# ooowedyn/InkLayer

Hardware: AMD Instinct MI355X
Metric: sketches/sec end-to-end (GroundingDINO+SAM) at 1024x1024 (higher is better)
Workload: dtype f16 (MFMA, f32 accumulate; f32 residual/norm/softmax; split-f16 = fp32-grade operands for patch-embed, neck, mask decoder)

## Files before the change

include/inklayer_hip.h:

```cpp
#ifndef INKLAYER_HIP_H
#define INKLAYER_HIP_H

#include <stdint.h>

#ifdef __cplusplus
extern "C" {
#endif

#define INK_ABI_VERSION 7
int ink_abi_version(void);

typedef struct InkGemm {
  const void* A;
  const void* W;
  const float* bias;
  const float* col_scale;
  const float* residual;
  const int32_t* row_map;
  void* C;
  int32_t M, N, K;
  int32_t lda, ldw, ldr, ldc;
  int32_t act;
  int32_t c_f16;
} InkGemm;
#define INK_ACT_NONE 0
#define INK_ACT_GELU 1
#define INK_ACT_RELU 2
int ink_gemm_f16(const InkGemm* p, void* stream);
int ink_gemm_set_variant(int32_t v);
int ink_gemm_query_variant(int32_t M, int32_t N, int32_t K);

int ink_layernorm_rows(const float* x, int64_t ldx, const float* gamma, const float* beta,
                       float eps, const int32_t* gather, int32_t rows_out, int32_t C,
                       void* out_f16, float* out_f32, int64_t ldo, int32_t act, int32_t split,
                       const float* add, int64_t ld_add, const int32_t* add_batch_rows, int32_t rows_per_batch,
                       void* stream);

int ink_add_cvt_f16(const float* a, const float* b, int64_t n_b, void* out_f16, int64_t n,
                    void* stream);
int ink_add_split_f16(const float* a, const float* b, int64_t n_b, void* out_f16, int64_t n, int32_t C,
                      void* stream);
int ink_add_f32(const float* a, const float* b, int64_t n_b, float* out, int64_t n, void* stream);

typedef struct InkAttn {
  const void* Q; const void* K; const void* V;
  void* O;
  int64_t ldq, ldk, ldv, ldo;
  int32_t n_batch, n_heads, n_q, n_k, head_dim;
  float scale;
  int32_t bias_mode;
  int32_t grid_w;
  const int32_t* q_batch_rows;
  const int32_t* kv_batch_rows;
  const float* rel_h; const float* rel_w;
  const void* rel_aug;
  const float* dense_bias; const float* dense_mask;
  int32_t n_mask; int32_t rel_f16;
  const int32_t* tok_rows;
  const void* pad_k; const void* pad_v;
} InkAttn;
int ink_flash_attn(const InkAttn* p, void* stream);

int ink_relpos_bias64_f16(const void* Q, int64_t ldq, const float* rel_pos_h, const float* rel_pos_w, int32_t n_batch,
                          int32_t n_heads, int32_t head_dim, float scale, void* out_h_f16, void* out_w_f16, void* stream);

int ink_relpos_bias(const void* Q, int64_t ldq, const float* rel_pos_h, const float* rel_pos_w,
                    int32_t S, int32_t n_batch, int32_t n_heads, int32_t head_dim, float scale,
                    const int32_t* tok_rows, float* out_h, float* out_w, void* out_aug_f16,
                    void* stream);

int ink_sam_patchify(const void* image_u8, int32_t h, int32_t w, int32_t L, int32_t P,
                     const float* mean3, const float* std3, int32_t chan_reverse, int32_t split,
                     void* out_f16, void* stream);

int ink_resize_bilinear_u8(const void* src_u8, int32_t h, int32_t w, void* dst_u8, int32_t oh, int32_t ow,
                           const int32_t* xbounds, const int32_t* xcoef, int32_t kx,
                           const int32_t* ybounds, const int32_t* ycoef, int32_t ky, void* tmp_u8,
                           void* stream);

int ink_im2col3x3_f16(const void* in_f16, int32_t B, int32_t H, int32_t W, int32_t C, void* out_f16,
                      void* stream);

int ink_sam_pe_encode(const float* coords01, const float* gauss, int32_t N, int32_t F,
                      const float* add, int32_t n_add, float* out, void* stream);

int ink_sam_prompt_tokens(const float* points, const int32_t* labels, int32_t n_pts, int32_t pad, const float* boxes,
                          const float* gauss, int32_t F, const float* point_emb, const float* not_a_point,
                          const float* out_tok, float input_size, int32_t P, float* out, void* stream);

int ink_sam_mask_embed(const float* mask, const float* emb, const int32_t* emb_rows, const float* params,
                       int32_t n_params, float eps, int32_t P, int32_t g, float* keys, void* split_f16, void* stream);

int ink_sam_mask_logits(const float* up, const float* hyper, int32_t n, int32_t g, int32_t C,
                        float* out, void* stream);

int ink_sam_postprocess(const float* low, int32_t n, int32_t S, int32_t L, int32_t in_h,
                        int32_t in_w, int32_t out_h, int32_t out_w, float thr, void* out_u8,
                        float* out_logits, void* stream);

int ink_ms_deform_attn_forward(const float* value, const int64_t* spatial_shapes_host,
                               const int64_t* level_start_index_host, const float* sampling_loc,
                               const float* attn_weight, int32_t B, int32_t S, int32_t M, int32_t C,
                               int32_t Q, int32_t L, int32_t P, int32_t im2col_step, float* out,
                               void* stream);

int ink_ms_deform_attn_forward_dev(const void* value, const int64_t* spatial_shapes,
                                   const int64_t* level_start_index, const void* sampling_loc,
                                   const void* attn_weight, int32_t dtype, int32_t B, int32_t S, int32_t M,
                                   int32_t C, int32_t Q, int32_t L, int32_t P, int32_t im2col_step,
                                   void* out, void* stream);
int ink_ms_deform_attn_backward_dev(const void* value, const int64_t* spatial_shapes,
                                    const int64_t* level_start_index, const void* sampling_loc,
                                    const void* attn_weight, const void* grad_output, int32_t dtype,
                                    int32_t B, int32_t S, int32_t M, int32_t C, int32_t Q, int32_t L,
                                    int32_t P, int32_t im2col_step, void* grad_value,
                                    void* grad_sampling_loc, void* grad_attn_weight, void* stream);

int ink_msda_fused(const void* value_f16, const float* proj, int64_t ldp, const float* ref,
                   int32_t ref_dim, int64_t ref_q_stride, int64_t ref_b_stride,
                   const int32_t* shapes_host, int32_t B, int32_t S, int32_t Q, void* out_f16,
                   void* stream);

int ink_swin_patchify(const void* image_u8, int32_t h, int32_t w, const float* mean3,
                      const float* std3, void* out_f16, void* stream);

int ink_layernorm_merge4(const float* x, int64_t ldx, const float* gamma, const float* beta, float eps,
                         const int32_t* gather4, int32_t rows, int32_t C, void* out_f16, void* stream);

int ink_groupnorm_nhwc(const float* x, int32_t B, int32_t T, int32_t C, int32_t G, const float* gamma,
                       const float* beta, float eps, float* stats_ws, float* out,
                       int64_t out_batch_stride, void* stream);

int ink_gather_rows(const float* x, int64_t ldx, int64_t x_batch_rows, const int32_t* idx,
                    int64_t idx_batch_stride, int32_t rows_per_batch, int32_t B, int32_t C,
                    void* out_f16, float* out_f32, void* stream);

int ink_biattn_fusion(const void* QV_f16, const void* KL_f16, int32_t B, int32_t S, int32_t T, int32_t E,
                      float scale, float* scores_ws, float* stats_ws, float* partial_ws, int32_t chunk,
                      void* out_v_f16, void* out_l_f16, void* stream);

int ink_attn_fewkeys(const void* Q, int64_t ldq, const void* K, int64_t ldk, const void* V, int64_t ldv,
                     int32_t B, int32_t n_q, int32_t n_k, int32_t n_heads, int32_t head_dim, float scale,
                     const uint8_t* blocked, const int32_t* q_batch_rows, const float* q_add, int32_t io_f32, void* O,
                     int64_t ldo, void* stream);

int ink_attn_fewq(const void* Q, int64_t ldq, const void* K, int64_t ldk, const void* V, int64_t ldv,
                  int32_t n_batch, int32_t n_q, int32_t n_k, int32_t n_heads, int32_t head_dim, float scale,
                  const int32_t* q_batch_rows, const int32_t* kv_batch_rows, const float* k_add, int32_t io_f32, void* O,
                  int64_t ldo, void* stream);

int ink_biattn_colstats(const float* scores, int32_t B, int32_t S, int32_t HT, float* part_ws, float* stats, void* stream);

int ink_fusion_fold_workspace(int32_t B, int32_t S, int64_t* out_floats);
int ink_fusion_fold(float* v_f32, int32_t B, int32_t S, const float* lnv_g, const float* lnv_b, float eps,
                    const float* text_k_f32, const float* text_vl_f32, int64_t ld_text, int32_t T, const void* Wq_f16,
                    const float* bq, const void* Wvv_f16, const float* bvv, const void* Wo_f16, const float* bo,
                    const float* gamma_v, float scale, float* ws, void* out_l_f16, const float* pos, void* out16_pos,
                    void* out16, void* stream);

int ink_sam_upscale_pack(const void* ws_f16, void* blob_f16, void* stream);
int ink_sam_upscale_tail(const float* u0, int64_t ld_tok, int32_t n, int32_t g, const float* ln_g, const float* ln_b, float eps,
                         const void* blob_f16, const float* b3, const float* hyper, int32_t n_masks, float* low,
                         void* stream);

int ink_proj256_ln_pack(const void* ws_f16, void* blob_f16, void* stream);
int ink_proj256_ln(const float* a_f32, const void* blob_f16, const float* bias, const float* res_f32,
                   const int32_t* res_batch_rows, int32_t rows_per_batch, const float* ln_g, const float* ln_b, float eps,
                   int64_t rows, float* out_f32, void* out_split_f16, void* stream);

int ink_ffn256_pack_bytes(int32_t hid, int32_t with_pre, int64_t* out_bytes);
int ink_ffn256_pack(const void* w1_f16, const float* b1, const void* w2_f16, int32_t hid, const void* wpre_f16, void* blob,
                    void* stream);
int ink_ffn256_fused(const void* x_f16, int64_t ldx, const float* res_f32, const void* blob, const float* b2,
                     const float* ln_g, const float* ln_b, float eps, int32_t M, int32_t hid, const float* pre_bias,
                     const float* pre_ln_g, const float* pre_ln_b, float* out_f32, void* stream);

int ink_topk_rowmax(const float* logits, int32_t B, int32_t S, int32_t T, int32_t K, int32_t* out_idx,
                    float* out_val, void* cand_ws, void* stream);

int ink_sine_embed4(const float* ref, const float* dim_t, int32_t N, void* out_f16, void* stream);

int ink_box_refine(const float* delta, int64_t ldd, const float* ref, int32_t N, int32_t ref_is_logit,
                   float* out, void* stream);

int ink_mask_cleanup_workspace_ints(int32_t n, int32_t H, int32_t W, int32_t k, int64_t* out_ints);
int ink_mask_cleanup(const void* masks_u8, int32_t n, int32_t H, int32_t W, int32_t k, int32_t area_threshold,
                     double aspect_threshold, void* tmp_a_u8, void* tmp_b_u8, int32_t* workspace, void* out_u8,
                     void* stream);

int ink_mask_sketch_iou_counts(const void* masks_u8, const void* sketch_rgb_u8, int32_t n, int32_t H, int32_t W,
                               void* bits_ws_u64, int32_t* counts, void* stream);

int ink_sam_amg_stats(const float* low, int32_t n, const int32_t* index, int32_t m, const int32_t* m_dev, int32_t S,
                      int32_t L, int32_t in_h, int32_t in_w, int32_t crop_h, int32_t crop_w, double thr, double offset,
                      int32_t x0, int32_t y0, int32_t orig_h, int32_t orig_w, int32_t* table, void* planes_u64,
                      float* out_logits, void* stream);

int ink_mask_rle_counts(const void* planes_u64, const int32_t* select, int32_t k, int32_t H, int32_t W,
                        int32_t* n_counts, void* stream);
int ink_mask_rle_write(const void* planes_u64, const int32_t* select, int32_t k, int32_t H, int32_t W,
                       const int32_t* offsets, int32_t* counts, void* stream);

int ink_mask_small_regions_workspace_ints(int32_t k, int32_t H, int32_t W, int64_t* out_ints);
int ink_mask_small_regions(const void* planes_u64, int32_t k, int32_t H, int32_t W, int32_t min_area, int32_t holes,
                           void* tmp_planes_u64, int32_t* workspace, void* out_planes_u64, int32_t* changed, void* stream);

int ink_box_nms(const float* boxes, const float* scores, int32_t n, float iou_threshold, void* workspace_u64,
                int32_t* keep, int32_t* n_keep, void* stream);

int ink_refine_sketch_planes(const void* rgb_u8, int32_t H, int32_t W, void* planes4_u64, int32_t* max_ws, void* stream);

int ink_bitplane_pack(const void* img_u8, int32_t n, int32_t H, int32_t W, int32_t thresh, void* planes_u64, void* stream);

int ink_refine_depth_samples(const void* mask_planes, int32_t n, const float* depth, const int32_t* pts_yx, int32_t P,
                             int32_t H, int32_t W, float* vals, void* inside_u8, void* stream);

int ink_refine_pair_tables(const void* mask_planes, const void* sketch_planes4, int32_t n, int32_t H, int32_t W,
                           const int32_t* rect, void* dil_ws_planes, int32_t* pair, int32_t* per_mask,
                           int32_t* sketch_area, void* stream);

int ink_refine_composite(const void* mask_planes, const int32_t* order, int32_t n_ranks, int32_t H, int32_t W,
                         void* label_u8, int32_t* hist256, void* stream);

int ink_refine_relabel_clean(const void* label_u8, const void* map256_u8, int32_t H, int32_t W, void* out_label_u8,
                             void* stream);

int ink_refine_grow_workspace(int32_t H, int32_t W, int64_t* plane_words, int64_t* cc_ints);
int ink_refine_grow(const void* label_u8, const void* sketch_planes4, int32_t H, int32_t W, void* planes_ws,
                    int32_t* cc_ws, int32_t* flags256, void* out_label_u8, int32_t* bbox256x4, int32_t* unl_yx,
                    int32_t unl_cap, int32_t* unl_count, void* stream);

int ink_refine_query_dists(const void* label_u8, const int32_t* q_yx, const void* cand256_bits, int32_t Q, int32_t H,
                           int32_t W, int32_t* d2_Qx256, void* stream);

int ink_refine_finalize(void* label_u8, const int32_t* assign_yxl, int32_t A, const void* sketch_planes4, int32_t H,
                        int32_t W, void* planes_ws3, void* extra_plane, int32_t* extra_count, void* stream);

int ink_host_sparse_sample(const uint8_t* rgb_u8, int32_t H, int32_t W, int32_t* out_yx, int32_t cap, int32_t* count);
int ink_host_assign_unlabeled(const int32_t* q_yx, int32_t Q, const int32_t* boxes, int32_t nb, const int32_t* box2mask,
                              const int32_t* d2, const uint8_t* nonempty, int32_t n_masks, int32_t* out_label);

int ink_depth_patchify(const void* image_u8, int32_t H, int32_t W, int32_t nh, int32_t nw, int32_t P, int32_t KP,
                       const double* mean3, const double* std3, int32_t chan_reverse, void* out_f16, void* stream);

int ink_resize_bilinear_ac_nhwc(const float* in, int32_t B, int32_t h, int32_t w, int32_t C, int32_t H, int32_t W,
                                float* out_f32, void* out_f16, void* stream);

int ink_im2col3x3_ex_f16(const void* in_f16, int32_t B, int32_t H, int32_t W, int32_t C, int32_t stride, int32_t relu,
                         void* out_f16, void* stream);

#ifdef __cplusplus
}
#endif
#endif
```

inklayer_amd/_lib.py:

```python
from __future__ import annotations

import ctypes as C
import os
from pathlib import Path

_LIB_PATH = Path(__file__).resolve().parent / "lib" / "libinklayer_hip.so"
_lib = None

c_void_p, c_int, c_i64, c_float = C.c_void_p, C.c_int32, C.c_int64, C.c_float


class InkGemm(C.Structure):
    _fields_ = [
        ("A", c_void_p), ("W", c_void_p), ("bias", c_void_p), ("col_scale", c_void_p),
        ("residual", c_void_p), ("row_map", c_void_p), ("C", c_void_p),
        ("M", c_int), ("N", c_int), ("K", c_int),
        ("lda", c_int), ("ldw", c_int), ("ldr", c_int), ("ldc", c_int),
        ("act", c_int), ("c_f16", c_int),
    ]


class InkAttn(C.Structure):
    _fields_ = [
        ("Q", c_void_p), ("K", c_void_p), ("V", c_void_p), ("O", c_void_p),
        ("ldq", c_i64), ("ldk", c_i64), ("ldv", c_i64), ("ldo", c_i64),
        ("n_batch", c_int), ("n_heads", c_int), ("n_q", c_int), ("n_k", c_int),
        ("head_dim", c_int), ("scale", c_float), ("bias_mode", c_int), ("grid_w", c_int),
        ("q_batch_rows", c_void_p), ("kv_batch_rows", c_void_p),
        ("rel_h", c_void_p), ("rel_w", c_void_p), ("rel_aug", c_void_p),
        ("dense_bias", c_void_p), ("dense_mask", c_void_p), ("n_mask", c_int), ("rel_f16", c_int),
        ("tok_rows", c_void_p), ("pad_k", c_void_p), ("pad_v", c_void_p),
    ]


SIGNATURES = {
    "ink_abi_version": [],
    "ink_gemm_f16": [C.POINTER(InkGemm), c_void_p],
    "ink_gemm_set_variant": [c_int],
    "ink_gemm_query_variant": [c_int, c_int, c_int],
    "ink_layernorm_rows": [c_void_p, c_i64, c_void_p, c_void_p, c_float, c_void_p, c_int, c_int,
                           c_void_p, c_void_p, c_i64, c_int, c_int, c_void_p, c_i64, c_void_p, c_int, c_void_p],
    "ink_add_split_f16": [c_void_p, c_void_p, c_i64, c_void_p, c_i64, c_int, c_void_p],
    "ink_add_cvt_f16": [c_void_p, c_void_p, c_i64, c_void_p, c_i64, c_void_p],
    "ink_add_f32": [c_void_p, c_void_p, c_i64, c_void_p, c_i64, c_void_p],
    "ink_flash_attn": [C.POINTER(InkAttn), c_void_p],
    "ink_sam_patchify": [c_void_p, c_int, c_int, c_int, c_int, C.POINTER(c_float), C.POINTER(c_float),
                         c_int, c_int, c_void_p, c_void_p],
    "ink_im2col3x3_f16": [c_void_p, c_int, c_int, c_int, c_int, c_void_p, c_void_p],
    "ink_resize_bilinear_u8": [c_void_p, c_int, c_int, c_void_p, c_int, c_int, c_void_p, c_void_p, c_int,
                               c_void_p, c_void_p, c_int, c_void_p, c_void_p],
    "ink_sam_pe_encode": [c_void_p, c_void_p, c_int, c_int, c_void_p, c_int, c_void_p, c_void_p],
    "ink_sam_mask_logits": [c_void_p, c_void_p, c_int, c_int, c_int, c_void_p, c_void_p],
    "ink_sam_prompt_tokens": [c_void_p, c_void_p, c_int, c_int, c_void_p, c_void_p, c_int, c_void_p, c_void_p,
                              c_void_p, c_float, c_int, c_void_p, c_void_p],
    "ink_sam_mask_embed": [c_void_p, c_void_p, c_void_p, c_void_p, c_int, c_float, c_int, c_int, c_void_p, c_void_p,
                           c_void_p],
    "ink_sam_postprocess": [c_void_p, c_int, c_int, c_int, c_int, c_int, c_int, c_int, c_float,
                            c_void_p, c_void_p, c_void_p],
    "ink_sam_amg_stats": [c_void_p, c_int, c_void_p, c_int, c_void_p, c_int, c_int, c_int, c_int, c_int, c_int, C.c_double,
                          C.c_double, c_int, c_int, c_int, c_int, c_void_p, c_void_p, c_void_p, c_void_p],
    "ink_mask_rle_counts": [c_void_p, c_void_p, c_int, c_int, c_int, c_void_p, c_void_p],
    "ink_mask_rle_write": [c_void_p, c_void_p, c_int, c_int, c_int, c_void_p, c_void_p, c_void_p],
    "ink_mask_small_regions_workspace_ints": [c_int, c_int, c_int, C.POINTER(c_i64)],
    "ink_mask_small_regions": [c_void_p, c_int, c_int, c_int, c_int, c_int, c_void_p, c_void_p, c_void_p, c_void_p,
                               c_void_p],
    "ink_box_nms": [c_void_p, c_void_p, c_int, c_float, c_void_p, c_void_p, c_void_p, c_void_p],
    "ink_ms_deform_attn_forward": [c_void_p, C.POINTER(c_i64), C.POINTER(c_i64), c_void_p, c_void_p, c_int,
                                   c_int, c_int, c_int, c_int, c_int, c_int, c_int, c_void_p, c_void_p],
    "ink_ms_deform_attn_forward_dev": [c_void_p, c_void_p, c_void_p, c_void_p, c_void_p, c_int, c_int, c_int, c_int,
                                       c_int, c_int, c_int, c_int, c_int, c_void_p, c_void_p],
    "ink_ms_deform_attn_backward_dev": [c_void_p, c_void_p, c_void_p, c_void_p, c_void_p, c_void_p, c_int, c_int, c_int,
                                        c_int, c_int, c_int, c_int, c_int, c_int, c_void_p, c_void_p, c_void_p,
                                        c_void_p],
    "ink_msda_fused": [c_void_p, c_void_p, c_i64, c_void_p, c_int, c_i64, c_i64, C.POINTER(c_int), c_int,
                       c_int, c_int, c_void_p, c_void_p],
    "ink_swin_patchify": [c_void_p, c_int, c_int, C.POINTER(c_float), C.POINTER(c_float), c_void_p, c_void_p],
    "ink_layernorm_merge4": [c_void_p, c_i64, c_void_p, c_void_p, c_float, c_void_p, c_int, c_int, c_void_p,
                             c_void_p],
    "ink_groupnorm_nhwc": [c_void_p, c_int, c_int, c_int, c_int, c_void_p, c_void_p, c_float, c_void_p,
                           c_void_p, c_i64, c_void_p],
    "ink_gather_rows": [c_void_p, c_i64, c_i64, c_void_p, c_i64, c_int, c_int, c_int, c_void_p, c_void_p,
                        c_void_p],
    "ink_biattn_fusion": [c_void_p, c_void_p, c_int, c_int, c_int, c_int, c_float, c_void_p, c_void_p,
                          c_void_p, c_int, c_void_p, c_void_p, c_void_p],
    "ink_biattn_colstats": [c_void_p, c_int, c_int, c_int, c_void_p, c_void_p, c_void_p],
    "ink_fusion_fold_workspace": [c_int, c_int, C.POINTER(c_i64)],
    "ink_relpos_bias64_f16": [c_void_p, c_i64, c_void_p, c_void_p, c_int, c_int, c_int, c_float, c_void_p, c_void_p, c_void_p],
    "ink_proj256_ln_pack": [c_void_p, c_void_p, c_void_p],
    "ink_proj256_ln": [c_void_p, c_void_p, c_void_p, c_void_p, c_void_p, c_int, c_void_p, c_void_p, c_float, c_i64, c_void_p,
                       c_void_p, c_void_p],
    "ink_sam_upscale_pack": [c_void_p, c_void_p, c_void_p],
    "ink_sam_upscale_tail": [c_void_p, c_i64, c_int, c_int, c_void_p, c_void_p, c_float, c_void_p, c_void_p, c_void_p,
                             c_int, c_void_p, c_void_p],
    "ink_ffn256_pack_bytes": [c_int, c_int, C.POINTER(c_i64)],
    "ink_ffn256_pack": [c_void_p, c_void_p, c_void_p, c_int, c_void_p, c_void_p, c_void_p],
    "ink_ffn256_fused": [c_void_p, c_i64, c_void_p, c_void_p, c_void_p, c_void_p, c_void_p, c_float, c_int, c_int,
                         c_void_p, c_void_p, c_void_p, c_void_p, c_void_p],
    "ink_fusion_fold": [c_void_p, c_int, c_int, c_void_p, c_void_p, c_float, c_void_p, c_void_p, c_i64, c_int, c_void_p,
                        c_void_p, c_void_p, c_void_p, c_void_p, c_void_p, c_void_p, c_float, c_void_p, c_void_p, c_void_p,
                        c_void_p, c_void_p, c_void_p],
    "ink_attn_fewkeys": [c_void_p, c_i64, c_void_p, c_i64, c_void_p, c_i64, c_int, c_int, c_int, c_int, c_int,
                         c_float, c_void_p, c_void_p, c_void_p, c_int, c_void_p, c_i64, c_void_p],
    "ink_attn_fewq": [c_void_p, c_i64, c_void_p, c_i64, c_void_p, c_i64, c_int, c_int, c_int, c_int, c_int,
                      c_float, c_void_p, c_void_p, c_void_p, c_int, c_void_p, c_i64, c_void_p],
    "ink_topk_rowmax": [c_void_p, c_int, c_int, c_int, c_int, c_void_p, c_void_p, c_void_p, c_void_p],
    "ink_sine_embed4": [c_void_p, c_void_p, c_int, c_void_p, c_void_p],
    "ink_box_refine": [c_void_p, c_i64, c_void_p, c_int, c_int, c_void_p, c_void_p],
    "ink_mask_cleanup_workspace_ints": [c_int, c_int, c_int, c_int, C.POINTER(c_i64)],
    "ink_mask_cleanup": [c_void_p, c_int, c_int, c_int, c_int, c_int, C.c_double, c_void_p, c_void_p, c_void_p,
                         c_void_p, c_void_p],
    "ink_mask_sketch_iou_counts": [c_void_p, c_void_p, c_int, c_int, c_int, c_void_p, c_void_p, c_void_p],
    "ink_refine_sketch_planes": [c_void_p, c_int, c_int, c_void_p, c_void_p, c_void_p],
    "ink_bitplane_pack": [c_void_p, c_int, c_int, c_int, c_int, c_void_p, c_void_p],
    "ink_refine_depth_samples": [c_void_p, c_int, c_void_p, c_void_p, c_int, c_int, c_int, c_void_p, c_void_p, c_void_p],
    "ink_refine_pair_tables": [c_void_p, c_void_p, c_int, c_int, c_int, c_void_p, c_void_p, c_void_p, c_void_p,
                               c_void_p, c_void_p],
    "ink_refine_composite": [c_void_p, c_void_p, c_int, c_int, c_int, c_void_p, c_void_p, c_void_p],
    "ink_refine_relabel_clean": [c_void_p, c_void_p, c_int, c_int, c_void_p, c_void_p],
    "ink_refine_grow_workspace": [c_int, c_int, C.POINTER(c_i64), C.POINTER(c_i64)],
    "ink_refine_grow": [c_void_p, c_void_p, c_int, c_int, c_void_p, c_void_p, c_void_p, c_void_p, c_void_p, c_void_p,
                        c_int, c_void_p, c_void_p],
    "ink_refine_query_dists": [c_void_p, c_void_p, c_void_p, c_int, c_int, c_int, c_void_p, c_void_p],
    "ink_refine_finalize": [c_void_p, c_void_p, c_int, c_void_p, c_int, c_int, c_void_p, c_void_p, c_void_p, c_void_p],
    "ink_host_sparse_sample": [c_void_p, c_int, c_int, c_void_p, c_int, c_void_p],
    "ink_host_assign_unlabeled": [c_void_p, c_int, c_void_p, c_int, c_void_p, c_void_p, c_void_p, c_int, c_void_p],
    "ink_depth_patchify": [c_void_p, c_int, c_int, c_int, c_int, c_int, c_int, C.POINTER(C.c_double), C.POINTER(C.c_double),
                           c_int, c_void_p, c_void_p],
    "ink_resize_bilinear_ac_nhwc": [c_void_p, c_int, c_int, c_int, c_int, c_int, c_int, c_void_p, c_void_p, c_void_p],
    "ink_im2col3x3_ex_f16": [c_void_p, c_int, c_int, c_int, c_int, c_int, c_int, c_void_p, c_void_p],
    "ink_relpos_bias": [c_void_p, c_i64, c_void_p, c_void_p, c_int, c_int, c_int, c_int, c_float,
                        c_void_p, c_void_p, c_void_p, c_void_p, c_void_p],
}


class InkLayerHipError(RuntimeError):
    pass


def lib_path() -> Path:
    return Path(os.environ.get("INKLAYER_HIP_LIB", _LIB_PATH))


def lib() -> C.CDLL:
    global _lib
    if _lib is None:
        p = lib_path()
        if not p.exists():
            raise InkLayerHipError(
                f"{p} not found: build it with `python -m inklayer_amd.build` "
                "(there is no CPU/eager fallback for the InkLayer hot path)")
        try:
            import torch
        except ImportError:
            pass
        l = C.CDLL(str(p))
        for name, argtypes in SIGNATURES.items():
            fn = getattr(l, name)
            fn.argtypes = argtypes
            fn.restype = C.c_int
        _lib = l
    return _lib


def check(rc: int, what: str) -> None:
    if rc != 0:
        raise InkLayerHipError(f"{what} failed: " + {1: "bad argument", 2: "HIP launch error"}.get(rc, str(rc)))
```

inklayer_amd/build.py:

```python
from __future__ import annotations

import os
import subprocess
import sys
from concurrent.futures import ThreadPoolExecutor
from pathlib import Path

ROOT = Path(__file__).resolve().parent
CSRC = ROOT / "csrc"
LIBDIR = ROOT / "lib"
OBJDIR = LIBDIR / "obj"
LIB = LIBDIR / "libinklayer_hip.so"
HIPCC = os.environ.get("HIPCC", "/opt/rocm/bin/hipcc")
FLAGS = ["--offload-arch=gfx950", "-O3", "-std=c++17", "-fPIC", "-ffp-contract=off",
         "-mllvm", "-amdgpu-mfma-vgpr-form",

         "-Wall", "-Wno-unused-function", "-Wno-unused-variable"]


def _newest_header() -> float:
    hs = list(CSRC.glob("*.h")) + list((ROOT.parent / "include").glob("*.h"))
    return max(h.stat().st_mtime for h in hs)


NO_SPILL = {"ffn_fused.hip", "proj_ln.hip", "amg.hip"}


def _check_no_spill(src: Path, remarks: str) -> None:
    name = None
    for line in remarks.splitlines():
        if "Function Name:" in line:
            name = line.split("Function Name:")[1].split("[")[0].strip()
        elif "ScratchSize [bytes/lane]:" in line:
            n = int(line.split("ScratchSize [bytes/lane]:")[1].split("[")[0])
            if n != 0:
                raise RuntimeError(f"{src.name}: kernel {name} spills ({n} bytes of scratch per lane) - the kernels of "
                                   f"this file must stay in registers (see NO_SPILL); reduce register pressure")


def _compile(src: Path, force: bool, hdr_time: float) -> Path:
    obj = OBJDIR / (src.stem + ".o")
    if (not force and obj.exists() and obj.stat().st_mtime > src.stat().st_mtime
            and obj.stat().st_mtime > hdr_time):
        return obj
    guard = src.name in NO_SPILL
    cmd = [HIPCC, *FLAGS, *(["-Rpass-analysis=kernel-resource-usage", "-fno-caret-diagnostics"] if guard else []), "-c", str(src), "-o", str(obj)]
    r = subprocess.run(cmd, capture_output=True, text=True)
    if r.returncode != 0:
        raise RuntimeError(f"hipcc failed for {src.name}:\n{r.stdout}\n{r.stderr}")
    err = r.stderr
    if guard:
        try:
            _check_no_spill(src, err)
        except RuntimeError:
            obj.unlink(missing_ok=True)
            raise
        err = "\n".join(l for l in err.splitlines()
                        if "kernel-resource-usage" not in l and not l.startswith("In file included from"))
    if err.strip():
        sys.stderr.write(err)
    return obj


def build(force: bool = False, verbose: bool = True) -> Path:
    OBJDIR.mkdir(parents=True, exist_ok=True)
    srcs = sorted(CSRC.glob("*.hip"))
    if not srcs:
        raise RuntimeError("no HIP sources found")
    hdr_time = _newest_header()
    with ThreadPoolExecutor(max_workers=min(8, len(srcs))) as ex:
        objs = list(ex.map(lambda s: _compile(s, force, hdr_time), srcs))
    if (force or not LIB.exists()
            or any(o.stat().st_mtime > LIB.stat().st_mtime for o in objs)):
        cmd = [HIPCC, "--offload-arch=gfx950", "-shared", "-fPIC", "-o", str(LIB),
               *map(str, objs)]
        r = subprocess.run(cmd, capture_output=True, text=True)
        if r.returncode != 0:
            raise RuntimeError(f"link failed:\n{r.stdout}\n{r.stderr}")
    if verbose:
        print(f"[inklayer_amd.build] {LIB} ({LIB.stat().st_size >> 10} KiB, {len(srcs)} sources)")
    return LIB


if __name__ == "__main__":
    build(force="--force" in sys.argv)
```

inklayer_amd/ops.py:

```python
from __future__ import annotations

import ctypes as C
from typing import Optional, Sequence, Tuple

import torch

from . import _lib
from ._lib import InkAttn, InkGemm, check

ACT = {None: 0, "none": 0, "gelu": 1, "relu": 2}
F16, F32 = torch.float16, torch.float32


_GEMM_TRACE = None


def set_gemm_trace(lst) -> None:
    global _GEMM_TRACE
    _GEMM_TRACE = lst


_ATTN_TRACE = None


def set_attn_trace(lst) -> None:
    global _ATTN_TRACE
    _ATTN_TRACE = lst


def tracing_off() -> bool:
    return _GEMM_TRACE is None and _ATTN_TRACE is None


_raw_stream = getattr(torch._C, "_cuda_getCurrentRawStream", None)
_cur_device = getattr(torch._C, "_cuda_getDevice", None)


def _stream() -> int:
    if _raw_stream is not None and _cur_device is not None:
        return _raw_stream(_cur_device())
    return torch.cuda.current_stream().cuda_stream


def own_f32(t: torch.Tensor, dev) -> torch.Tensor:
    t = t.detach().to(dev, F32).contiguous()
    if t.untyped_storage().nbytes() > t.numel() * t.element_size():
        t = t.clone()
    return t


def _p(t: Optional[torch.Tensor]) -> Optional[int]:
    if t is None:
        return None
    assert t.is_cuda, "InkLayer HIP ops need GPU tensors (no CPU fallback)"
    return t.data_ptr()


def gemm(a: torch.Tensor, w: torch.Tensor, bias: Optional[torch.Tensor] = None, *,
         act: Optional[str] = None, residual: Optional[torch.Tensor] = None,
         col_scale: Optional[torch.Tensor] = None, row_map: Optional[torch.Tensor] = None,
         out: Optional[torch.Tensor] = None, out_dtype: torch.dtype = F32,
         out_rows: Optional[int] = None) -> torch.Tensor:
    assert a.dtype == F16 and w.dtype == F16
    assert a.dim() == 2 and w.dim() == 2 and a.stride(1) == 1 and w.stride(1) == 1
    M, K = a.shape
    N = w.shape[0]
    assert w.shape[1] == K
    p = InkGemm()
    if out is None:
        rows = out_rows if out_rows is not None else M
        out = torch.empty((rows, N), device=a.device, dtype=out_dtype)
    assert out.dim() == 2 and out.stride(1) == 1 and out.shape[1] == N
    p.A, p.W, p.C = a.data_ptr(), w.data_ptr(), out.data_ptr()
    p.bias, p.col_scale = _p(bias), _p(col_scale)
    p.residual, p.row_map = _p(residual), _p(row_map)
    if bias is not None:
        assert bias.dtype == F32 and bias.numel() == N
    if col_scale is not None:
        assert col_scale.dtype == F32 and col_scale.numel() == N
    if residual is not None:
        assert residual.dtype == F32 and residual.stride(1) == 1 and residual.shape[1] == N
        p.ldr = residual.stride(0)
    if row_map is not None:
        assert row_map.dtype == torch.int32 and row_map.numel() == M
    p.M, p.N, p.K = M, N, K
    p.lda, p.ldw, p.ldc = a.stride(0), w.stride(0), out.stride(0)
    p.act = ACT[act]
    p.c_f16 = 1 if out.dtype == F16 else 0
    assert out.dtype in (F16, F32)
    if _GEMM_TRACE is None:
        check(_lib.lib().ink_gemm_f16(C.byref(p), _stream()), "ink_gemm_f16")
    else:
        e0, e1 = torch.cuda.Event(enable_timing=True), torch.cuda.Event(enable_timing=True)
        e0.record()
        check(_lib.lib().ink_gemm_f16(C.byref(p), _stream()), "ink_gemm_f16")
        e1.record()
        _GEMM_TRACE.append((2.0 * M * N * K, e0, e1, (M, N, K, act or '-', 'res' if residual is not None else '-',
                                                      'map' if row_map is not None else '-', 'f16' if p.c_f16 else 'f32')))
    return out


def layernorm_rows(x: torch.Tensor, gamma: Optional[torch.Tensor], beta: Optional[torch.Tensor],
                   eps: float, *, gather: Optional[torch.Tensor] = None,
                   out_dtype: torch.dtype = F16, out: Optional[torch.Tensor] = None,
                   out2: Optional[torch.Tensor] = None, act: Optional[str] = None,
                   split: bool = False, add: Optional[torch.Tensor] = None,
                   add_batch_rows: Optional[torch.Tensor] = None, rows_per_batch: int = 0,
                   split_f32: Optional[torch.Tensor] = None) -> torch.Tensor:
    assert x.dtype == F32 and x.dim() == 2 and x.stride(1) == 1
    Cdim = x.shape[1]
    rows = gather.numel() if gather is not None else x.shape[0]
    wcols = 3 * Cdim if split else Cdim
    if split:
        assert out_dtype == F16 and out2 is None
    if out is None:
        out = torch.empty((rows, wcols), device=x.device, dtype=out_dtype)
    assert out.shape == (rows, wcols) and out.stride(1) == 1
    oh = out.data_ptr() if out.dtype == F16 else None
    of = out.data_ptr() if out.dtype == F32 else None
    if out2 is not None:
        assert out2.shape == out.shape and out2.stride(0) == out.stride(0) and out2.dtype != out.dtype
        if out2.dtype == F16:
            oh = out2.data_ptr()
        else:
            of = out2.data_ptr()
    if split_f32 is not None:
        assert split and out.stride(0) == 3 * Cdim and split_f32.dtype == F32 and split_f32.is_contiguous()
        assert tuple(split_f32.shape) == (rows, Cdim)
        of = split_f32.data_ptr()
    if gather is not None:
        assert gather.dtype == torch.int32
    if add is not None:
        assert gather is None and add.dtype == F32 and add.dim() == 2 and add.stride(1) == 1 and add.shape[1] == Cdim
        if add_batch_rows is not None:
            assert add_batch_rows.dtype == torch.int32 and add_batch_rows.is_cuda and rows_per_batch > 0
            assert add_batch_rows.numel() * rows_per_batch == rows
        else:
            rows_per_batch = rows
    check(_lib.lib().ink_layernorm_rows(x.data_ptr(), x.stride(0), _p(gamma), _p(beta), eps,
                                        _p(gather), rows, Cdim, oh, of, out.stride(0), ACT[act], int(split),
                                        _p(add), add.stride(0) if add is not None else 0, _p(add_batch_rows),
                                        rows_per_batch, _stream()), "ink_layernorm_rows")
    return out


def add_cvt_f16(a: torch.Tensor, b: Optional[torch.Tensor] = None,
                out: Optional[torch.Tensor] = None) -> torch.Tensor:
    assert a.dtype == F32 and a.is_contiguous()
    nb = 0
    if b is not None:
        assert b.dtype == F32 and b.is_contiguous() and a.numel() % b.numel() == 0
        nb = b.numel()
    if out is None:
        out = torch.empty(a.shape, device=a.device, dtype=F16)
    assert out.dtype == F16 and out.is_contiguous() and out.numel() == a.numel()
    check(_lib.lib().ink_add_cvt_f16(a.data_ptr(), _p(b), nb, out.data_ptr(), a.numel(), _stream()),
          "ink_add_cvt_f16")
    return out


def add_split_f16(a: torch.Tensor, b: Optional[torch.Tensor] = None) -> torch.Tensor:
    assert a.dtype == F32 and a.is_contiguous() and a.dim() == 2
    nb = 0
    if b is not None:
        assert b.dtype == F32 and b.is_contiguous() and a.numel() % b.numel() == 0
        nb = b.numel()
    R, Cn = a.shape
    out = torch.empty((R, 3 * Cn), device=a.device, dtype=F16)
    check(_lib.lib().ink_add_split_f16(a.data_ptr(), _p(b), nb, out.data_ptr(), a.numel(), Cn, _stream()),
          "ink_add_split_f16")
    return out


def split_weight(w32: torch.Tensor) -> torch.Tensor:
    w32 = w32.to(torch.float32)
    hi = w32.to(F16)
    lo = ((w32 - hi.to(torch.float32)) * 64.0).to(F16)
    return torch.cat([hi, (hi.to(torch.float32) / 64.0).to(F16), lo], dim=-1).contiguous()


def add_f32(a: torch.Tensor, b: torch.Tensor, out: Optional[torch.Tensor] = None) -> torch.Tensor:
    assert a.dtype == F32 and b.dtype == F32 and a.is_contiguous() and b.is_contiguous()
    assert a.numel() % b.numel() == 0
    if out is None:
        out = torch.empty(a.shape, device=a.device, dtype=F32)
    assert out.is_contiguous() and out.numel() == a.numel()
    check(_lib.lib().ink_add_f32(a.data_ptr(), b.data_ptr(), b.numel(), out.data_ptr(), a.numel(),
                                 _stream()), "ink_add_f32")
    return out


def flash_attn(q: torch.Tensor, k: torch.Tensor, v: torch.Tensor, *, n_batch: int, n_heads: int,
               head_dim: int, scale: float, n_q: Optional[int] = None, n_k: Optional[int] = None,
               rel_h: Optional[torch.Tensor] = None, rel_w: Optional[torch.Tensor] = None,
               rel_aug: Optional[torch.Tensor] = None, grid_w: int = 0,
               dense_bias: Optional[torch.Tensor] = None, dense_mask: Optional[torch.Tensor] = None,
               q_batch_rows: Optional[torch.Tensor] = None,
               kv_batch_rows: Optional[torch.Tensor] = None,
               tok_rows: Optional[torch.Tensor] = None, pad_k: Optional[torch.Tensor] = None,
               pad_v: Optional[torch.Tensor] = None,
               out: Optional[torch.Tensor] = None) -> torch.Tensor:
    for t in (q, k, v):
        assert t.dtype == F16 and t.dim() == 2 and t.stride(1) == 1 and t.is_cuda
    if n_q is None:
        n_q = q.shape[0] // n_batch
    if n_k is None:
        n_k = k.shape[0] // n_batch
    if tok_rows is not None:
        assert rel_aug is not None and out is not None and n_q == n_k
        assert tok_rows.dtype == torch.int32 and tok_rows.is_cuda and tok_rows.numel() == n_batch * n_q
        for t in (pad_k, pad_v):
            assert t is not None and t.dtype == F16 and t.is_contiguous() and t.numel() == n_heads * head_dim
        assert out.dtype == F16 and out.stride(1) == 1
        assert out.shape[0] * out.stride(0) * 2 < 2 ** 31 and q.shape[0] * q.stride(0) * 2 < 2 ** 32
    else:
        if out is None:
            out = torch.empty((n_batch * n_q, n_heads * head_dim), device=q.device, dtype=F16)
        assert out.dtype == F16 and out.shape[0] == n_batch * n_q and out.stride(1) == 1
    p = InkAttn()
    p.Q, p.K, p.V, p.O = q.data_ptr(), k.data_ptr(), v.data_ptr(), out.data_ptr()
    p.ldq, p.ldk, p.ldv, p.ldo = q.stride(0), k.stride(0), v.stride(0), out.stride(0)
    p.n_batch, p.n_heads, p.n_q, p.n_k, p.head_dim = n_batch, n_heads, n_q, n_k, head_dim
    p.scale = scale
    p.grid_w = grid_w
    for name, t in (("q_batch_rows", q_batch_rows), ("kv_batch_rows", kv_batch_rows)):
        if t is not None:
            assert t.dtype == torch.int32 and t.numel() == n_batch and t.is_cuda
            setattr(p, name, t.data_ptr())
    if dense_bias is not None:
        assert dense_bias.dtype == F32 and dense_bias.is_contiguous() and dense_bias.shape == (n_heads, n_q, 64)
        p.bias_mode, p.dense_bias = 3, dense_bias.data_ptr()
        if dense_mask is not None:
            assert dense_mask.dtype == F32 and dense_mask.is_contiguous() and dense_mask.shape[1:] == (n_q, 64)
            p.dense_mask, p.n_mask = dense_mask.data_ptr(), dense_mask.shape[0]
    elif rel_aug is not None:
        assert rel_aug.dtype == F16 and rel_aug.is_contiguous()
        p.bias_mode, p.rel_aug = 2, rel_aug.data_ptr()
        if tok_rows is not None:
            p.tok_rows, p.pad_k, p.pad_v = tok_rows.data_ptr(), pad_k.data_ptr(), pad_v.data_ptr()
    elif rel_h is not None:
        assert rel_h.dtype == rel_w.dtype and rel_h.dtype in (F32, F16)
        assert rel_h.is_contiguous() and rel_w.is_contiguous()
        p.bias_mode, p.rel_h, p.rel_w = 1, rel_h.data_ptr(), rel_w.data_ptr()
        p.rel_f16 = int(rel_h.dtype == F16)
    else:
        p.bias_mode = 0
    if _ATTN_TRACE is None:
        check(_lib.lib().ink_flash_attn(C.byref(p), _stream()), "ink_flash_attn")
    else:
        e0, e1 = torch.cuda.Event(enable_timing=True), torch.cuda.Event(enable_timing=True)
        e0.record()
        check(_lib.lib().ink_flash_attn(C.byref(p), _stream()), "ink_flash_attn")
        e1.record()
        _ATTN_TRACE.append((n_batch, n_heads, n_q, n_k, head_dim, int(p.bias_mode), int(out.shape[0]), e0, e1))
    return out


def relpos_bias(q: torch.Tensor, rel_pos_h: torch.Tensor, rel_pos_w: torch.Tensor, *, S: int,
                n_batch: int, n_heads: int, head_dim: int, scale: float, out=None,
                tok_rows: Optional[torch.Tensor] = None, f16_tables: bool = False):
    assert q.dtype == F16 and q.stride(1) == 1
    assert rel_pos_h.dtype == F32 and rel_pos_h.is_contiguous()
    assert rel_pos_w.dtype == F32 and rel_pos_w.is_contiguous()
    assert rel_pos_h.shape == (2 * S - 1, head_dim)
    n = n_batch * n_heads * S * S
    fn = _lib.lib().ink_relpos_bias
    if S == 64 and f16_tables:
        oh, ow = out if out is not None else (torch.empty((n, 64), device=q.device, dtype=F16),
                                              torch.empty((n, 64), device=q.device, dtype=F16))
        assert oh.dtype == F16 and ow.dtype == F16 and oh.numel() >= n * 64 and ow.numel() >= n * 64
        check(_lib.lib().ink_relpos_bias64_f16(q.data_ptr(), q.stride(0), rel_pos_h.data_ptr(), rel_pos_w.data_ptr(), n_batch,
                                               n_heads, head_dim, scale, oh.data_ptr(), ow.data_ptr(), _stream()),
              "ink_relpos_bias64_f16")
        return oh, ow
    if S == 64:
        oh, ow = out if out is not None else (torch.empty((n, 64), device=q.device, dtype=F32),
                                              torch.empty((n, 64), device=q.device, dtype=F32))
        assert oh.numel() >= n * 64 and ow.numel() >= n * 64
        check(fn(q.data_ptr(), q.stride(0), rel_pos_h.data_ptr(), rel_pos_w.data_ptr(), S, n_batch,
                 n_heads, head_dim, scale, None, oh.data_ptr(), ow.data_ptr(), None, _stream()),
              "ink_relpos_bias")
        return oh, ow
    aug = out if out is not None else torch.empty((n, 32), device=q.device, dtype=F16)
    assert aug.numel() >= n * 32
    if tok_rows is not None:
        assert tok_rows.dtype == torch.int32 and tok_rows.is_cuda and tok_rows.numel() == n_batch * S * S
    check(fn(q.data_ptr(), q.stride(0), rel_pos_h.data_ptr(), rel_pos_w.data_ptr(), S, n_batch,
             n_heads, head_dim, scale, tok_rows.data_ptr() if tok_rows is not None else None,
             None, None, aug.data_ptr(), _stream()), "ink_relpos_bias")
    return aug


def resize_bilinear_u8(image_u8: torch.Tensor, oh: int, ow: int, out: Optional[torch.Tensor] = None) -> torch.Tensor:
    from .resize import plan_for
    assert image_u8.dtype == torch.uint8 and image_u8.is_cuda and image_u8.is_contiguous()
    h, w, c = image_u8.shape
    assert c == 3
    if (oh, ow) == (h, w):
        return image_u8
    pl = plan_for(h, w, oh, ow, image_u8.device)
    if out is None:
        out = torch.empty((oh, ow, 3), device=image_u8.device, dtype=torch.uint8)
    assert out.dtype == torch.uint8 and out.is_contiguous() and tuple(out.shape) == (oh, ow, 3)
    ptr = lambda t: t.data_ptr() if t is not None else None
    check(_lib.lib().ink_resize_bilinear_u8(image_u8.data_ptr(), h, w, out.data_ptr(), oh, ow, ptr(pl.xb), ptr(pl.xk),
                                            pl.kx, ptr(pl.yb), ptr(pl.yk), pl.ky, ptr(pl.tmp), _stream()),
          "ink_resize_bilinear_u8")
    return out


def sam_patchify(image_u8: torch.Tensor, L: int, P: int, mean: Sequence[float],
                 std: Sequence[float], chan_reverse: bool, out: torch.Tensor, split: bool = False) -> torch.Tensor:
    assert image_u8.dtype == torch.uint8 and image_u8.is_cuda and image_u8.is_contiguous()
    h, w, c = image_u8.shape
    assert c == 3 and out.dtype == F16 and out.is_contiguous()
    assert out.numel() == (L // P) ** 2 * 3 * P * P * (3 if split else 1)
    m = (C.c_float * 3)(*mean)
    s = (C.c_float * 3)(*std)
    check(_lib.lib().ink_sam_patchify(image_u8.data_ptr(), h, w, L, P, m, s, int(chan_reverse), int(split),
                                      out.data_ptr(), _stream()), "ink_sam_patchify")
    return out


def im2col3x3(x: torch.Tensor, B: int, H: int, W: int, out: Optional[torch.Tensor] = None) -> torch.Tensor:
    assert x.dtype == F16 and x.is_contiguous() and x.shape[0] == B * H * W
    Cn = x.shape[1]
    if out is None:
        out = torch.empty((B * H * W, 9 * Cn), device=x.device, dtype=F16)
    check(_lib.lib().ink_im2col3x3_f16(x.data_ptr(), B, H, W, Cn, out.data_ptr(), _stream()),
          "ink_im2col3x3_f16")
    return out


def sam_pe_encode(coords01: torch.Tensor, gauss: torch.Tensor,
                  add: Optional[torch.Tensor] = None, out: Optional[torch.Tensor] = None) -> torch.Tensor:
    assert coords01.dtype == F32 and coords01.is_contiguous() and coords01.shape[-1] == 2
    assert gauss.dtype == F32 and gauss.is_contiguous() and gauss.shape[0] == 2
    N, Fd = coords01.numel() // 2, gauss.shape[1]
    if out is None:
        out = torch.empty((N, 2 * Fd), device=coords01.device, dtype=F32)
    assert out.dtype == F32 and out.is_contiguous() and tuple(out.shape) == (N, 2 * Fd)
    n_add = 0
    if add is not None:
        assert add.dtype == F32 and add.is_contiguous() and add.shape[-1] == 2 * Fd
        n_add = add.numel() // (2 * Fd)
    check(_lib.lib().ink_sam_pe_encode(coords01.data_ptr(), gauss.data_ptr(), N, Fd, _p(add), n_add,
                                       out.data_ptr(), _stream()), "ink_sam_pe_encode")
    return out


def sam_prompt_tokens(gauss: torch.Tensor, point_emb: torch.Tensor, not_a_point: torch.Tensor, out_tok: torch.Tensor,
                      input_size: float, P: int, points: Optional[torch.Tensor] = None,
                      labels: Optional[torch.Tensor] = None, boxes: Optional[torch.Tensor] = None, pad: bool = False,
                      out: Optional[torch.Tensor] = None) -> torch.Tensor:
    Fd = gauss.shape[1]
    assert gauss.dtype == F32 and gauss.is_contiguous() and gauss.shape[0] == 2
    for t, n in ((point_emb, 4), (not_a_point, 1), (out_tok, 5)):
        assert t.dtype == F32 and t.is_contiguous() and t.numel() == n * 2 * Fd
    n_pts = 0
    if points is not None:
        assert labels is not None and points.dtype == F32 and labels.dtype == torch.int32
        assert points.is_contiguous() and labels.is_contiguous() and points.dim() == 3 and points.shape[0] == P
        n_pts = points.shape[1]
        assert tuple(points.shape) == (P, n_pts, 2) and tuple(labels.shape) == (P, n_pts)
    if boxes is not None:
        assert boxes.dtype == F32 and boxes.is_contiguous() and tuple(boxes.shape) == (P, 4)
    NT = 5 + n_pts + int(pad) + (2 if boxes is not None else 0)
    if out is None:
        out = torch.empty((P, NT, 2 * Fd), device=gauss.device, dtype=F32)
    assert out.dtype == F32 and out.is_contiguous() and tuple(out.shape) == (P, NT, 2 * Fd)
    check(_lib.lib().ink_sam_prompt_tokens(_p(points), _p(labels), n_pts, int(pad), _p(boxes), _p(gauss), Fd,
                                           _p(point_emb), _p(not_a_point), _p(out_tok),
                                           float(input_size), P, _p(out), _stream()), "ink_sam_prompt_tokens")
    return out


SAM_MASK_EMBED_PARAMS = 4684


def sam_mask_embed(mask: torch.Tensor, emb: torch.Tensor, emb_rows: torch.Tensor, params: torch.Tensor, eps: float,
                   split: bool = False):
    assert mask.dtype == F32 and mask.is_contiguous() and mask.dim() == 4 and mask.shape[1] == 1
    P, S = mask.shape[0], mask.shape[2]
    assert mask.shape[3] == S and S % 4 == 0
    g = S // 4
    assert emb.dtype == F32 and emb.is_contiguous() and emb.dim() == 2 and emb.shape[1] == 256
    assert emb_rows.dtype == torch.int32 and emb_rows.is_cuda and emb_rows.numel() == P
    assert params.dtype == F32 and params.is_contiguous() and params.numel() == SAM_MASK_EMBED_PARAMS
    keys = torch.empty((P * g * g, 256), device=mask.device, dtype=F32)
    ks = torch.empty((P * g * g, 768), device=mask.device, dtype=F16) if split else None
    check(_lib.lib().ink_sam_mask_embed(_p(mask), _p(emb), _p(emb_rows), _p(params),
                                        params.numel(), eps, P, g, _p(keys), _p(ks), _stream()),
          "ink_sam_mask_embed")
    return (keys, ks) if split else keys


def sam_mask_logits(up: torch.Tensor, hyper: torch.Tensor, n: int, g: int) -> torch.Tensor:
    assert up.dtype == F32 and up.is_contiguous() and hyper.dtype == F32 and hyper.is_contiguous()
    Cn = hyper.shape[1]
    assert up.numel() == n * g * g * 16 * Cn
    out = torch.empty((n, 4 * g, 4 * g), device=up.device, dtype=F32)
    check(_lib.lib().ink_sam_mask_logits(up.data_ptr(), hyper.data_ptr(), n, g, Cn, out.data_ptr(),
                                         _stream()), "ink_sam_mask_logits")
    return out


def sam_postprocess(low: torch.Tensor, L: int, input_hw: Tuple[int, int], orig_hw: Tuple[int, int],
                    thr: float = 0.0, want_logits: bool = False):
    assert low.dtype == F32 and low.is_contiguous() and low.dim() == 3
    n, S, _ = low.shape
    oh, ow = orig_hw
    out = torch.empty((n, oh, ow), device=low.device, dtype=torch.uint8)
    lg = torch.empty((n, oh, ow), device=low.device, dtype=F32) if want_logits else None
    check(_lib.lib().ink_sam_postprocess(low.data_ptr(), n, S, L, input_hw[0], input_hw[1], oh, ow,
                                         thr, out.data_ptr(), _p(lg), _stream()),
          "ink_sam_postprocess")
    return (out, lg) if want_logits else out


NMS_MAX_BOXES = 4096


def sam_amg_stats(low: torch.Tensor, L: int, input_hw: Tuple[int, int], crop_hw: Tuple[int, int], thr: float,
                  offset: float, xy0: Tuple[int, int] = (0, 0), orig_hw: Optional[Tuple[int, int]] = None,
                  index: Optional[torch.Tensor] = None, count: Optional[torch.Tensor] = None,
                  want_logits: bool = False):
    assert low.dtype == F32 and low.is_contiguous() and low.dim() == 3
    n, S, _ = low.shape
    ch, cw = crop_hw
    oh, ow = orig_hw if orig_hw is not None else crop_hw
    if index is not None:
        assert index.dtype == torch.int32 and index.is_cuda and index.is_contiguous() and index.dim() == 1
    if count is not None:
        assert count.dtype == torch.int32 and count.is_cuda and count.numel() == 1
    m = n if index is None else index.numel()
    hp = -(-oh // 64)
    table = torch.empty((m, 8), device=low.device, dtype=torch.int32)
    planes = torch.empty((m, ow, hp), device=low.device, dtype=torch.int64)
    lg = torch.empty((m, ch, cw), device=low.device, dtype=F32) if want_logits else None
    if m > 0:
        check(_lib.lib().ink_sam_amg_stats(low.data_ptr(), n, _p(index), m, _p(count), S, L, input_hw[0], input_hw[1],
                                           ch, cw, thr, offset, xy0[0], xy0[1], oh, ow, table.data_ptr(),
                                           planes.data_ptr(), _p(lg), _stream()), "ink_sam_amg_stats")
    return (table, planes, lg) if want_logits else (table, planes)


def mask_rle(planes: torch.Tensor, H: int, W: int, select: Optional[torch.Tensor] = None):
    assert planes.dtype == torch.int64 and planes.is_cuda and planes.is_contiguous()
    assert planes.dim() == 3 and tuple(planes.shape[1:]) == (W, -(-H // 64))
    if select is not None:
        assert select.dtype == torch.int32 and select.is_cuda and select.is_contiguous() and select.dim() == 1
    k = planes.shape[0] if select is None else select.numel()
    if k == 0:
        return []
    nc = torch.empty((k,), device=planes.device, dtype=torch.int32)
    check(_lib.lib().ink_mask_rle_counts(planes.data_ptr(), _p(select), k, H, W, nc.data_ptr(), _stream()),
          "ink_mask_rle_counts")
    sizes = nc.cpu()
    ends = torch.cumsum(sizes.long(), 0)
    total = int(ends[-1])
    assert total < 2 ** 31
    offs = (ends - sizes).to(torch.int32).to(planes.device)
    counts = torch.empty((total,), device=planes.device, dtype=torch.int32)
    check(_lib.lib().ink_mask_rle_write(planes.data_ptr(), _p(select), k, H, W, offs.data_ptr(), counts.data_ptr(),
                                        _stream()), "ink_mask_rle_write")
    return [c.tolist() for c in torch.split(counts.cpu(), sizes.tolist())]


def box_nms(boxes: torch.Tensor, scores: torch.Tensor, iou_threshold: float) -> torch.Tensor:
    assert boxes.dtype == F32 and boxes.is_cuda and boxes.is_contiguous() and boxes.dim() == 2 and boxes.shape[1] == 4
    assert scores.dtype == F32 and scores.is_cuda and scores.is_contiguous() and scores.shape == boxes.shape[:1]
    n = boxes.shape[0]
    if n > NMS_MAX_BOXES:
        raise ValueError(f"box_nms serves at most {NMS_MAX_BOXES} boxes, got {n}")
    if n == 0:
        return torch.empty((0,), device=boxes.device, dtype=torch.int64)
    ws = torch.empty((n * (-(-n // 64) + 3),), device=boxes.device, dtype=torch.int64)
    keep = torch.empty((n + 1,), device=boxes.device, dtype=torch.int32)
    check(_lib.lib().ink_box_nms(boxes.data_ptr(), scores.data_ptr(), n, iou_threshold, ws.data_ptr(), keep.data_ptr(),
                                 keep[n:].data_ptr(), _stream()), "ink_box_nms")
    host = keep.cpu()
    return host[:int(host[n])].long().to(boxes.device)


def pack_col_planes(masks: torch.Tensor) -> torch.Tensor:
    assert masks.is_cuda and masks.dim() == 3 and masks.dtype in (torch.bool, torch.uint8)
    k, H, W = masks.shape
    t = masks.to(torch.uint8).transpose(1, 2).contiguous()
    planes = torch.empty((k, W, -(-H // 64)), device=masks.device, dtype=torch.int64)
    if k:
        check(_lib.lib().ink_bitplane_pack(t.data_ptr(), k, W, H, 0, planes.data_ptr(), _stream()), "ink_bitplane_pack")
    return planes


def remove_small_regions(planes: torch.Tensor, H: int, W: int, min_area: int, max_workspace_bytes: int = 1 << 29,
                         modes: Sequence[str] = ("holes", "islands")) -> Tuple[torch.Tensor, torch.Tensor]:
    assert planes.dtype == torch.int64 and planes.is_cuda and planes.is_contiguous()
    assert planes.dim() == 3 and tuple(planes.shape[1:]) == (W, -(-H // 64))
    k = planes.shape[0]
    out = torch.empty_like(planes)
    changed = torch.zeros((k,), device=planes.device, dtype=torch.int32)
    if k == 0:
        return out, changed.bool()
    L = _lib.lib()
    one = C.c_int64(0)
    check(L.ink_mask_small_regions_workspace_ints(1, H, W, C.byref(one)), "ink_mask_small_regions_workspace_ints")
    chunk = max(1, min(k, max_workspace_bytes // (4 * one.value)))
    need = C.c_int64(0)
    check(L.ink_mask_small_regions_workspace_ints(chunk, H, W, C.byref(need)), "ink_mask_small_regions_workspace_ints")
    ws = torch.empty((need.value,), device=planes.device, dtype=torch.int32)
    tmp = torch.empty_like(planes[:chunk])
    flag = torch.empty((chunk,), device=planes.device, dtype=torch.int32)
    for a in range(0, k, chunk):
        n = min(chunk, k - a)
        src, dst = planes[a:a + n], out[a:a + n]
        for j, mode in enumerate(modes):
            assert mode in ("holes", "islands")
            holes = int(mode == "holes")
            check(L.ink_mask_small_regions((dst if j else src).data_ptr(), n, H, W, int(min_area), holes,
                                           tmp.data_ptr(), ws.data_ptr(), dst.data_ptr(), flag.data_ptr(), _stream()),
                  "ink_mask_small_regions")
            changed[a:a + n] |= flag[:n]
    return out, changed.bool()


_MSDA_DTYPE = {F32: 0, torch.float64: 1}


def _msda_check(value: torch.Tensor, spatial_shapes, level_start_index, sampling_loc: torch.Tensor,
                attn_weight: torch.Tensor, im2col_step: int, *grads: torch.Tensor):
    ss = spatial_shapes if isinstance(spatial_shapes, torch.Tensor) else torch.as_tensor(spatial_shapes)
    ls = level_start_index if isinstance(level_start_index, torch.Tensor) else torch.as_tensor(level_start_index)
    floats = (value, sampling_loc, attn_weight, *grads)
    if value.dtype not in _MSDA_DTYPE:
        raise ValueError(f"ms_deform_attn: value must be float32 or float64, got {value.dtype}")
    if any(t.dtype != value.dtype for t in floats):
        raise ValueError("ms_deform_attn: value, sampling_loc, attn_weight (and grad_output) must share one dtype, got "
                         + ", ".join(str(t.dtype) for t in floats))
    if ss.dtype != torch.int64 or ls.dtype != torch.int64:
        raise ValueError(f"ms_deform_attn: spatial_shapes / level_start_index must be int64, got {ss.dtype} / {ls.dtype}")
    if not all(t.is_cuda for t in floats):
        raise ValueError("ms_deform_attn: value, sampling_loc, attn_weight must be GPU tensors (no CPU path)")
    if not all(t.is_contiguous() for t in (*floats, ss, ls)):
        raise ValueError("ms_deform_attn: every tensor must be contiguous")
    if value.dim() != 4 or sampling_loc.dim() != 6 or sampling_loc.shape[-1] != 2:
        raise ValueError("ms_deform_attn: value must be [B,S,M,C] and sampling_loc [B,Q,M,L,P,2]")
    B, S, M, Cn = value.shape
    _, Q, _, L, P, _ = sampling_loc.shape
    if (tuple(sampling_loc.shape[:3]) != (B, Q, M) or tuple(attn_weight.shape) != (B, Q, M, L, P)
            or tuple(ss.shape) != (L, 2) or tuple(ls.shape) != (L,)):
        raise ValueError("ms_deform_attn: inconsistent shapes of value / spatial_shapes / level_start_index / "
                         "sampling_loc / attn_weight")
    if any(tuple(g.shape) != (B, Q, M * Cn) for g in grads):
        raise ValueError(f"ms_deform_attn: grad_output must be [B,Q,M*C] = {(B, Q, M * Cn)}")
    step = min(B, im2col_step)
    if im2col_step <= 0 or B % step != 0:
        raise ValueError(f"ms_deform_attn: im2col_step ({im2col_step}) must divide batch ({B})")
    for t, name in ((ss, "spatial_shapes"), (ls, "level_start_index")):
        if t.is_cuda and t.device != value.device:
            raise ValueError(f"ms_deform_attn: {name} is on {t.device}, value on {value.device}")
    return ss, ls, (B, S, M, Cn, Q, L, P)


def _msda_device_tables(ss: torch.Tensor, ls: torch.Tensor, S: int, dev) -> Tuple[torch.Tensor, torch.Tensor]:
    if ss.is_cuda and ls.is_cuda:
        return ss, ls
    if ss.is_cuda or ls.is_cuda:
        raise ValueError("ms_deform_attn: spatial_shapes and level_start_index must both be host or both be device tensors")
    hw = [int(h) * int(w) for h, w in ss.tolist()]
    starts = [sum(hw[:i]) for i in range(len(hw))]
    if min(int(v) for v in ss.reshape(-1).tolist()) <= 0 or sum(hw) != S or ls.tolist() != starts:
        raise ValueError(f"ms_deform_attn: spatial_shapes {ss.tolist()} / level_start_index {ls.tolist()} do not "
                         f"describe the {S} rows of value")
    return ss.to(dev), ls.to(dev)


def ms_deform_attn_forward(value: torch.Tensor, spatial_shapes, level_start_index,
                           sampling_loc: torch.Tensor, attn_weight: torch.Tensor,
                           im2col_step: int = 64) -> torch.Tensor:
    ss, ls, (B, S, M, Cn, Q, L, P) = _msda_check(value, spatial_shapes, level_start_index, sampling_loc, attn_weight,
                                                 im2col_step)
    out = torch.empty((B, Q, M * Cn), device=value.device, dtype=value.dtype)
    if not ss.is_cuda and not ls.is_cuda and value.dtype == F32 and Cn == 32 and L <= 8:
        sl = [int(v) for v in ss.reshape(-1).tolist()]
        ll = [int(v) for v in ls.tolist()]
        check(_lib.lib().ink_ms_deform_attn_forward(
            value.data_ptr(), (C.c_int64 * len(sl))(*sl), (C.c_int64 * len(ll))(*ll), sampling_loc.data_ptr(),
            attn_weight.data_ptr(), B, S, M, Cn, Q, L, P, im2col_step, out.data_ptr(), _stream()),
            "ink_ms_deform_attn_forward")
        return out
    ss, ls = _msda_device_tables(ss, ls, S, value.device)
    check(_lib.lib().ink_ms_deform_attn_forward_dev(
        value.data_ptr(), ss.data_ptr(), ls.data_ptr(), sampling_loc.data_ptr(), attn_weight.data_ptr(),
        _MSDA_DTYPE[value.dtype], B, S, M, Cn, Q, L, P, im2col_step, out.data_ptr(), _stream()),
        "ink_ms_deform_attn_forward_dev")
    return out


def ms_deform_attn_backward(value: torch.Tensor, spatial_shapes, level_start_index, sampling_loc: torch.Tensor,
                            attn_weight: torch.Tensor, grad_output: torch.Tensor, im2col_step: int = 64):
    ss, ls, (B, S, M, Cn, Q, L, P) = _msda_check(value, spatial_shapes, level_start_index, sampling_loc, attn_weight,
                                                 im2col_step, grad_output)
    ss, ls = _msda_device_tables(ss, ls, S, value.device)
    grad_value = torch.empty_like(value)
    grad_loc = torch.empty_like(sampling_loc)
    grad_aw = torch.empty_like(attn_weight)
    check(_lib.lib().ink_ms_deform_attn_backward_dev(
        value.data_ptr(), ss.data_ptr(), ls.data_ptr(), sampling_loc.data_ptr(), attn_weight.data_ptr(),
        grad_output.data_ptr(), _MSDA_DTYPE[value.dtype], B, S, M, Cn, Q, L, P, im2col_step, grad_value.data_ptr(),
        grad_loc.data_ptr(), grad_aw.data_ptr(), _stream()), "ink_ms_deform_attn_backward_dev")
    return grad_value, grad_loc, grad_aw


class _MSDeformAttnFunction(torch.autograd.Function):

    @staticmethod
    def forward(ctx, value, spatial_shapes, level_start_index, sampling_loc, attn_weight, im2col_step):
        ctx.im2col_step = im2col_step
        ctx.save_for_backward(value, spatial_shapes, level_start_index, sampling_loc, attn_weight)
        return ms_deform_attn_forward(value, spatial_shapes, level_start_index, sampling_loc, attn_weight, im2col_step)

    @staticmethod
    @torch.autograd.function.once_differentiable
    def backward(ctx, grad_output):
        value, spatial_shapes, level_start_index, sampling_loc, attn_weight = ctx.saved_tensors
        gv, gl, ga = ms_deform_attn_backward(value, spatial_shapes, level_start_index, sampling_loc, attn_weight,
                                             grad_output.contiguous(), ctx.im2col_step)
        return gv, None, None, gl, ga, None


def ms_deform_attn(value: torch.Tensor, spatial_shapes, level_start_index, sampling_loc: torch.Tensor,
                   attn_weight: torch.Tensor, im2col_step: int = 64) -> torch.Tensor:
    ss = spatial_shapes if isinstance(spatial_shapes, torch.Tensor) else torch.as_tensor(spatial_shapes)
    ls = level_start_index if isinstance(level_start_index, torch.Tensor) else torch.as_tensor(level_start_index)
    return _MSDeformAttnFunction.apply(value, ss, ls, sampling_loc, attn_weight, im2col_step)


def msda_fused(value16: torch.Tensor, proj: torch.Tensor, ref: torch.Tensor, shapes: Sequence[Tuple[int, int]],
               B: int, Q: int, ref_batched: bool, out: Optional[torch.Tensor] = None) -> torch.Tensor:
    assert value16.dtype == F16 and value16.is_contiguous() and proj.dtype == F32 and proj.stride(1) == 1
    assert ref.dtype == F32 and ref.is_contiguous()
    S = value16.shape[0] // B
    d = ref.shape[-1]
    if out is None:
        out = torch.empty((B * Q, 256), device=value16.device, dtype=F16)
    flat = [v for hw in shapes for v in hw]
    check(_lib.lib().ink_msda_fused(value16.data_ptr(), proj.data_ptr(), proj.stride(0), ref.data_ptr(), d, d,
                                    Q * d if ref_batched else 0, (C.c_int32 * 8)(*flat), B, S, Q,
                                    out.data_ptr(), _stream()), "ink_msda_fused")
    return out


def swin_patchify(image_u8: torch.Tensor, mean: Sequence[float], std: Sequence[float], out: torch.Tensor):
    assert image_u8.dtype == torch.uint8 and image_u8.is_cuda and image_u8.is_contiguous()
    h, w, c = image_u8.shape
    assert c == 3 and out.dtype == F16 and out.is_contiguous() and out.numel() == -(-h // 4) * -(-w // 4) * 64
    check(_lib.lib().ink_swin_patchify(image_u8.data_ptr(), h, w, (C.c_float * 3)(*mean), (C.c_float * 3)(*std),
                                       out.data_ptr(), _stream()), "ink_swin_patchify")
    return out


def layernorm_merge4(x: torch.Tensor, gamma, beta, eps: float, gather4: torch.Tensor,
                     out: Optional[torch.Tensor] = None) -> torch.Tensor:
    assert x.dtype == F32 and x.stride(1) == 1 and gather4.dtype == torch.int32 and gather4.is_contiguous()
    rows, Cn = gather4.shape[0], x.shape[1]
    if out is None:
        out = torch.empty((rows, 4 * Cn), device=x.device, dtype=F16)
    assert out.dtype == F16 and out.is_contiguous() and tuple(out.shape) == (rows, 4 * Cn)
    check(_lib.lib().ink_layernorm_merge4(x.data_ptr(), x.stride(0), gamma.data_ptr(), beta.data_ptr(), eps,
                                          gather4.data_ptr(), rows, Cn, out.data_ptr(), _stream()),
          "ink_layernorm_merge4")
    return out


def groupnorm_nhwc(x: torch.Tensor, B: int, T: int, G: int, gamma, beta, eps: float, out: torch.Tensor,
                   out_batch_stride: int) -> None:
    assert x.dtype == F32 and x.is_contiguous() and out.dtype == F32
    Cn = x.shape[1]
    ws = torch.empty(B * G * 2, device=x.device, dtype=F32)
    check(_lib.lib().ink_groupnorm_nhwc(x.data_ptr(), B, T, Cn, G, gamma.data_ptr(), beta.data_ptr(), eps,
                                        ws.data_ptr(), out.data_ptr(), out_batch_stride, _stream()),
          "ink_groupnorm_nhwc")


def gather_rows(x: torch.Tensor, idx: torch.Tensor, B: int, rows_per_batch: int, *, x_batch_rows: int,
                idx_batch_stride: int, out_dtype=F16, out: Optional[torch.Tensor] = None) -> torch.Tensor:
    assert x.dtype == F32 and x.stride(1) == 1 and idx.dtype == torch.int32 and idx.is_cuda
    Cn = x.shape[1]
    if out is None:
        out = torch.empty((B * rows_per_batch, Cn), device=x.device, dtype=out_dtype)
    out_dtype = out.dtype
    assert out_dtype in (F16, F32) and out.is_contiguous() and tuple(out.shape) == (B * rows_per_batch, Cn)
    oh = out.data_ptr() if out_dtype == F16 else None
    of = out.data_ptr() if out_dtype == F32 else None
    check(_lib.lib().ink_gather_rows(x.data_ptr(), x.stride(0), x_batch_rows, idx.data_ptr(), idx_batch_stride,
                                     rows_per_batch, B, Cn, oh, of, _stream()), "ink_gather_rows")
    return out


def biattn_fusion(qv16: torch.Tensor, kl16: torch.Tensor, B: int, S: int, T: int, scale: float,
                  chunk: int = 128):
    assert qv16.dtype == F16 and qv16.is_contiguous() and kl16.dtype == F16 and kl16.is_contiguous()
    E = qv16.shape[1] // 2
    dev = qv16.device
    nchunk = -(-S // chunk)
    scores = torch.empty(B * S * 4 * T, device=dev, dtype=F32)
    stats = torch.empty(B * 4 * T * 2, device=dev, dtype=F32)
    partial = torch.empty(B * 4 * nchunk * T * 256, device=dev, dtype=F32)
    out_v = torch.empty((B * S, E), device=dev, dtype=F16)
    out_l = torch.empty((B * T, E), device=dev, dtype=F16)
    check(_lib.lib().ink_biattn_fusion(qv16.data_ptr(), kl16.data_ptr(), B, S, T, E, scale, scores.data_ptr(),
                                       stats.data_ptr(), partial.data_ptr(), chunk, out_v.data_ptr(),
                                       out_l.data_ptr(), _stream()), "ink_biattn_fusion")
    return out_v, out_l


def fusion_fold(v: torch.Tensor, B: int, S: int, lnv_g: torch.Tensor, lnv_b: torch.Tensor, eps: float,
                text_kv: torch.Tensor, T: int, Wqv: torch.Tensor, bqv: torch.Tensor, Wo: torch.Tensor, bo: torch.Tensor,
                gamma_v: torch.Tensor, scale: float, pos: Optional[torch.Tensor] = None,
                out16_pos: Optional[torch.Tensor] = None, out16: Optional[torch.Tensor] = None) -> torch.Tensor:
    for t in (out16, out16_pos):
        assert t is None or (t.dtype == F16 and t.is_contiguous() and tuple(t.shape) == (B * S, 256))
    assert out16_pos is None or (pos is not None and pos.dtype == F32 and pos.is_contiguous() and tuple(pos.shape) == (S, 256))
    assert v.dtype == F32 and v.is_contiguous() and tuple(v.shape) == (B * S, 256)
    assert text_kv.dtype == F32 and text_kv.stride(1) == 1 and tuple(text_kv.shape) == (B * T, 2048)
    assert Wqv.dtype == F16 and Wqv.is_contiguous() and tuple(Wqv.shape) == (2048, 256) and bqv.dtype == F32
    assert Wo.dtype == F16 and Wo.is_contiguous() and tuple(Wo.shape) == (256, 1024)
    need = C.c_int64(0)
    check(_lib.lib().ink_fusion_fold_workspace(B, S, C.byref(need)), "ink_fusion_fold_workspace")
    ws = torch.empty(need.value, device=v.device, dtype=F32)
    out_l = torch.empty((B * T, 1024), device=v.device, dtype=F16)
    check(_lib.lib().ink_fusion_fold(v.data_ptr(), B, S, lnv_g.data_ptr(), lnv_b.data_ptr(), eps, text_kv.data_ptr(),
                                     text_kv[:, 1024:].data_ptr(), text_kv.stride(0), T, Wqv.data_ptr(), bqv.data_ptr(),
                                     Wqv[1024:].data_ptr(), bqv[1024:].data_ptr(), Wo.data_ptr(), bo.data_ptr(),
                                     gamma_v.data_ptr(), scale, ws.data_ptr(), out_l.data_ptr(), _p(pos), _p(out16_pos),
                                     _p(out16), _stream()),
          "ink_fusion_fold")
    return out_l


def proj256_ln_pack(ws: torch.Tensor) -> torch.Tensor:
    assert ws.dtype == F16 and ws.is_contiguous() and tuple(ws.shape) == (256, 384)
    blob = torch.empty(3 * 64 * 64 * 8, device=ws.device, dtype=F16)
    check(_lib.lib().ink_proj256_ln_pack(ws.data_ptr(), blob.data_ptr(), _stream()), "ink_proj256_ln_pack")
    return blob


def proj256_ln(a: torch.Tensor, blob: torch.Tensor, bias: torch.Tensor, res: torch.Tensor, ln_g: torch.Tensor,
               ln_b: torch.Tensor, eps: float, *, res_batch_rows: Optional[torch.Tensor] = None, rows_per_batch: int = 0,
               want_f32: bool = True, want_split: bool = True):
    R = int(a.shape[0])
    assert a.dtype == F32 and a.is_contiguous() and tuple(a.shape) == (R, 128)
    assert blob.dtype == F16 and blob.numel() == 3 * 64 * 64 * 8
    assert res.dtype == F32 and res.is_contiguous() and res.shape[1] == 256
    assert all(t.dtype == F32 and t.is_contiguous() and t.numel() == 256 for t in (bias, ln_g, ln_b))
    if res_batch_rows is not None:
        assert res_batch_rows.dtype == torch.int32 and res_batch_rows.is_cuda and rows_per_batch > 0
        assert res_batch_rows.numel() * rows_per_batch == R
    else:
        assert res.shape[0] == R
    of = torch.empty((R, 256), device=a.device, dtype=F32) if want_f32 else None
    osp = torch.empty((R, 768), device=a.device, dtype=F16) if want_split else None
    check(_lib.lib().ink_proj256_ln(a.data_ptr(), blob.data_ptr(), bias.data_ptr(), res.data_ptr(), _p(res_batch_rows),
                                    rows_per_batch, ln_g.data_ptr(), ln_b.data_ptr(), eps, R, _p(of), _p(osp), _stream()),
          "ink_proj256_ln")
    return of, osp


def sam_upscale_pack(ws: torch.Tensor) -> torch.Tensor:
    assert ws.dtype == F16 and ws.is_contiguous() and tuple(ws.shape) == (128, 192)
    blob = torch.empty(4 * 12 * 64 * 8, device=ws.device, dtype=F16)
    check(_lib.lib().ink_sam_upscale_pack(ws.data_ptr(), blob.data_ptr(), _stream()), "ink_sam_upscale_pack")
    return blob


def sam_upscale_tail(u0: torch.Tensor, n: int, g: int, ln_g: torch.Tensor, ln_b: torch.Tensor, eps: float,
                     blob: torch.Tensor, b3: torch.Tensor, hyper: torch.Tensor) -> torch.Tensor:
    if u0.shape[1] == 64:
        assert u0.is_contiguous() and u0.shape[0] == n * g * g * 4
        u0 = u0.view(n * g * g, 256)
    assert u0.dtype == F32 and u0.stride(1) == 1 and tuple(u0.shape) == (n * g * g, 256) and u0.stride(0) % 4 == 0
    assert blob.dtype == F16 and blob.numel() == 4 * 12 * 64 * 8 and b3.dtype == F32 and b3.numel() == 128
    assert hyper.dtype == F32 and hyper.is_contiguous() and hyper.dim() == 3 and hyper.shape[0] == n and hyper.shape[2] == 32
    assert ln_g.dtype == F32 and ln_b.dtype == F32 and ln_g.numel() == 64 and ln_b.numel() == 64
    M = hyper.shape[1]
    low = torch.empty((n, M, 4 * g, 4 * g), device=u0.device, dtype=F32)
    check(_lib.lib().ink_sam_upscale_tail(_p(u0), u0.stride(0), n, g, _p(ln_g), _p(ln_b), eps, _p(blob), _p(b3), _p(hyper), M,
                                          _p(low), _stream()), "ink_sam_upscale_tail")
    return low


def ffn256_pack(w1: torch.Tensor, b1: torch.Tensor, w2: torch.Tensor, w_pre: Optional[torch.Tensor] = None) -> torch.Tensor:
    hid = int(w1.shape[0])
    assert w1.dtype == F16 and w2.dtype == F16 and w1.is_contiguous() and w2.is_contiguous()
    assert tuple(w1.shape) == (hid, 256) and tuple(w2.shape) == (256, hid)
    assert b1.dtype == F32 and b1.is_contiguous() and b1.numel() == hid
    assert w_pre is None or (w_pre.dtype == F16 and w_pre.is_contiguous() and tuple(w_pre.shape) == (256, 256))
    need = C.c_int64(0)
    check(_lib.lib().ink_ffn256_pack_bytes(hid, int(w_pre is not None), C.byref(need)), "ink_ffn256_pack_bytes")
    blob = torch.empty(need.value // 2, device=w1.device, dtype=F16)
    check(_lib.lib().ink_ffn256_pack(w1.data_ptr(), b1.data_ptr(), w2.data_ptr(), hid, _p(w_pre), blob.data_ptr(), _stream()),
          "ink_ffn256_pack")
    return blob


def ffn256_fused(x16: torch.Tensor, res: torch.Tensor, blob: torch.Tensor, hid: int, b2: torch.Tensor,
                 ln_g: torch.Tensor, ln_b: torch.Tensor, eps: float, out: Optional[torch.Tensor] = None,
                 pre: Optional[Tuple[torch.Tensor, torch.Tensor, torch.Tensor]] = None) -> torch.Tensor:
    M = int(x16.shape[0])
    assert x16.dtype == F16 and x16.stride(1) == 1 and x16.shape[1] == 256
    assert res.dtype == F32 and res.is_contiguous() and tuple(res.shape) == (M, 256)
    need = C.c_int64(0)
    check(_lib.lib().ink_ffn256_pack_bytes(hid, int(pre is not None), C.byref(need)), "ink_ffn256_pack_bytes")
    assert blob.dtype == F16 and blob.numel() * 2 == need.value and b2.dtype == F32
    assert b2.numel() == 256 and ln_g.numel() == 256 and ln_b.numel() == 256 and ln_g.dtype == F32 and ln_b.dtype == F32
    if pre is not None:
        assert all(t.dtype == F32 and t.is_contiguous() and t.numel() == 256 for t in pre)
    if out is None:
        out = torch.empty_like(res)
    assert out.dtype == F32 and out.is_contiguous() and tuple(out.shape) == (M, 256)
    pb, pg, pe = pre if pre is not None else (None, None, None)
    check(_lib.lib().ink_ffn256_fused(x16.data_ptr(), x16.stride(0), res.data_ptr(), blob.data_ptr(), b2.data_ptr(),
                                      ln_g.data_ptr(), ln_b.data_ptr(), eps, M, hid, _p(pb), _p(pg), _p(pe), out.data_ptr(),
                                      _stream()), "ink_ffn256_fused")
    return out


def attn_fewkeys(q: torch.Tensor, k: torch.Tensor, v: torch.Tensor, *, B: int, n_heads: int, head_dim: int,
                 scale: float, blocked: Optional[torch.Tensor] = None, n_q: Optional[int] = None,
                 q_batch_rows: Optional[torch.Tensor] = None, q_add: Optional[torch.Tensor] = None) -> torch.Tensor:
    io = q.dtype
    for t in (q, k, v):
        assert t.dtype == io and io in (F16, F32) and t.dim() == 2 and t.stride(1) == 1
    if n_q is None:
        n_q = q.shape[0] // B
    n_k = k.shape[0] // B
    out = torch.empty((B * n_q, n_heads * head_dim), device=q.device, dtype=io)
    if blocked is not None:
        assert blocked.dtype == torch.uint8 and blocked.is_contiguous() and blocked.shape == (n_q, n_k)
    if q_batch_rows is not None:
        assert q_batch_rows.dtype == torch.int32 and q_batch_rows.numel() == B and q_batch_rows.is_cuda
    if q_add is not None:
        assert q_add.dtype == F32 and q_add.is_contiguous() and tuple(q_add.shape) == (n_q, n_heads * head_dim)
    check(_lib.lib().ink_attn_fewkeys(q.data_ptr(), q.stride(0), k.data_ptr(), k.stride(0), v.data_ptr(),
                                      v.stride(0), B, n_q, n_k, n_heads, head_dim, scale, _p(blocked),
                                      _p(q_batch_rows), _p(q_add), int(io == F32), out.data_ptr(), out.stride(0), _stream()),
          "ink_attn_fewkeys")
    return out


def attn_fewq(q: torch.Tensor, k: torch.Tensor, v: torch.Tensor, *, n_batch: int, n_heads: int, head_dim: int,
              scale: float, n_q: int, n_k: int, q_batch_rows: Optional[torch.Tensor] = None,
              kv_batch_rows: Optional[torch.Tensor] = None, k_add: Optional[torch.Tensor] = None) -> torch.Tensor:
    io = q.dtype
    for t in (q, k, v):
        assert t.dtype == io and io in (F16, F32) and t.dim() == 2 and t.stride(1) == 1
    out = torch.empty((n_batch * n_q, n_heads * head_dim), device=q.device, dtype=io)
    if k_add is not None:
        assert io == F32 and k_add.dtype == F32 and k_add.is_contiguous() and tuple(k_add.shape) == (n_k, n_heads * head_dim)
    check(_lib.lib().ink_attn_fewq(q.data_ptr(), q.stride(0), k.data_ptr(), k.stride(0), v.data_ptr(), v.stride(0),
                                   n_batch, n_q, n_k, n_heads, head_dim, scale, _p(q_batch_rows),
                                   _p(kv_batch_rows), _p(k_add), int(io == F32), out.data_ptr(), out.stride(0), _stream()),
          "ink_attn_fewq")
    return out


def topk_rowmax(logits: torch.Tensor, K: int, want_values: bool = False):
    assert logits.dtype == F32 and logits.is_contiguous() and logits.dim() == 3
    B, S, T = logits.shape
    idx = torch.empty((B, K), device=logits.device, dtype=torch.int32)
    val = torch.empty((B, K), device=logits.device, dtype=F32) if want_values else None
    nchunk = -(-S // 16384)
    ws = torch.empty((B * nchunk * K,), device=logits.device, dtype=torch.int64) if nchunk > 1 else None
    check(_lib.lib().ink_topk_rowmax(logits.data_ptr(), B, S, T, K, idx.data_ptr(), _p(val), _p(ws), _stream()),
          "ink_topk_rowmax")
    return (idx, val) if want_values else idx


def sine_embed4(ref: torch.Tensor, dim_t: torch.Tensor, out: Optional[torch.Tensor] = None) -> torch.Tensor:
    assert ref.dtype == F32 and ref.is_contiguous() and ref.shape[-1] == 4 and dim_t.numel() == 128
    N = ref.numel() // 4
    if out is None:
        out = torch.empty((N, 512), device=ref.device, dtype=F16)
    assert out.dtype == F16 and out.is_contiguous() and tuple(out.shape) == (N, 512)
    check(_lib.lib().ink_sine_embed4(ref.data_ptr(), dim_t.data_ptr(), N, out.data_ptr(), _stream()),
          "ink_sine_embed4")
    return out


def box_refine(delta: torch.Tensor, ref: torch.Tensor, ref_is_logit: bool = False,
               out: Optional[torch.Tensor] = None) -> torch.Tensor:
    assert delta.dtype == F32 and delta.stride(1) == 1 and ref.dtype == F32 and ref.is_contiguous()
    N = ref.numel() // 4
    if out is None:
        out = torch.empty_like(ref)
    assert out.dtype == F32 and out.is_contiguous() and out.shape == ref.shape
    check(_lib.lib().ink_box_refine(delta.data_ptr(), delta.stride(0), ref.data_ptr(), N, int(ref_is_logit),
                                    out.data_ptr(), _stream()), "ink_box_refine")
    return out


def mask_cleanup(masks_u8: torch.Tensor, k: int, area_threshold: int = 500, aspect_threshold: float = 1.1,
                 out: Optional[torch.Tensor] = None) -> torch.Tensor:
    assert masks_u8.dtype == torch.uint8 and masks_u8.is_cuda and masks_u8.is_contiguous() and masks_u8.dim() == 3
    n, H, W = masks_u8.shape
    if out is None:
        out = torch.empty_like(masks_u8)
    if n == 0:
        return out
    assert out.dtype == torch.uint8 and out.is_contiguous() and out.shape == masks_u8.shape
    need = C.c_int64(0)
    check(_lib.lib().ink_mask_cleanup_workspace_ints(n, H, W, k, C.byref(need)), "ink_mask_cleanup_workspace_ints")
    ws = torch.empty(need.value, device=masks_u8.device, dtype=torch.int32)
    ta, tb = torch.empty_like(masks_u8), torch.empty_like(masks_u8)
    check(_lib.lib().ink_mask_cleanup(masks_u8.data_ptr(), n, H, W, k, area_threshold, float(aspect_threshold),
                                      ta.data_ptr(), tb.data_ptr(), ws.data_ptr(), out.data_ptr(), _stream()),
          "ink_mask_cleanup")
    out._ink_overflow_flag = ws[:1]
    return out


def mask_sketch_iou_counts(masks_u8: torch.Tensor, sketch_rgb_u8: torch.Tensor) -> torch.Tensor:
    assert masks_u8.dtype == torch.uint8 and masks_u8.is_cuda and masks_u8.is_contiguous() and masks_u8.dim() == 3
    n, H, W = masks_u8.shape
    assert sketch_rgb_u8.dtype == torch.uint8 and sketch_rgb_u8.is_cuda and sketch_rgb_u8.is_contiguous()
    assert tuple(sketch_rgb_u8.shape) == (H, W, 3), "masks and sketch have the same size on this path"
    counts = torch.empty((n, n, 2), device=masks_u8.device, dtype=torch.int32)
    if n == 0:
        return counts
    bits = torch.empty((n, (H * W + 63) // 64), device=masks_u8.device, dtype=torch.int64)
    check(_lib.lib().ink_mask_sketch_iou_counts(masks_u8.data_ptr(), sketch_rgb_u8.data_ptr(), n, H, W,
                                                bits.data_ptr(), counts.data_ptr(), _stream()),
          "ink_mask_sketch_iou_counts")
    return counts


def depth_patchify(image_u8: torch.Tensor, nh: int, nw: int, P: int, KP: int, mean: Sequence[float],
                   std: Sequence[float], chan_reverse: bool) -> torch.Tensor:
    assert image_u8.dtype == torch.uint8 and image_u8.is_cuda and image_u8.is_contiguous() and image_u8.shape[2] == 3
    H, W = int(image_u8.shape[0]), int(image_u8.shape[1])
    out = torch.empty(((nh // P) * (nw // P), 3 * KP), device=image_u8.device, dtype=F16)
    check(_lib.lib().ink_depth_patchify(image_u8.data_ptr(), H, W, nh, nw, P, KP, (C.c_double * 3)(*mean),
                                        (C.c_double * 3)(*std), int(chan_reverse), out.data_ptr(), _stream()),
          "ink_depth_patchify")
    return out


def resize_bilinear_ac(x: torch.Tensor, B: int, h: int, w: int, H: int, W: int, out_dtype=F32) -> torch.Tensor:
    assert x.dtype == F32 and x.is_contiguous() and x.shape[0] == B * h * w
    Cn = x.shape[1]
    out = torch.empty((B * H * W, Cn), device=x.device, dtype=out_dtype)
    check(_lib.lib().ink_resize_bilinear_ac_nhwc(x.data_ptr(), B, h, w, Cn, H, W,
                                                 out.data_ptr() if out_dtype == F32 else None,
                                                 out.data_ptr() if out_dtype == F16 else None, _stream()),
          "ink_resize_bilinear_ac_nhwc")
    return out


def im2col3x3_ex(x: torch.Tensor, B: int, H: int, W: int, stride: int = 1, relu: bool = False) -> torch.Tensor:
    assert x.dtype == F16 and x.is_contiguous() and x.shape[0] == B * H * W
    Cn = x.shape[1]
    OH, OW = (H - 1) // stride + 1, (W - 1) // stride + 1
    out = torch.empty((B * OH * OW, 9 * Cn), device=x.device, dtype=F16)
    check(_lib.lib().ink_im2col3x3_ex_f16(x.data_ptr(), B, H, W, Cn, stride, int(relu), out.data_ptr(), _stream()),
          "ink_im2col3x3_ex_f16")
    return out
```

inklayer_amd/sam.py:

```python
from __future__ import annotations

import math
from dataclasses import dataclass
from typing import Dict, List, Optional, Sequence, Tuple

import numpy as np
import torch

from . import ops
from ._lru import LRU

F16, F32 = torch.float16, torch.float32


@dataclass
class SamConfig:
    embed_dim: int = 1280
    depth: int = 32
    num_heads: int = 16
    global_attn_indexes: Tuple[int, ...] = (7, 15, 23, 31)
    window_size: int = 14
    img_size: int = 1024
    patch_size: int = 16
    mlp_ratio: float = 4.0
    prompt_embed_dim: int = 256
    dec_depth: int = 2
    dec_heads: int = 8
    dec_mlp_dim: int = 2048
    num_mask_tokens: int = 4
    pixel_mean: Tuple[float, ...] = (123.675, 116.28, 103.53)
    pixel_std: Tuple[float, ...] = (58.395, 57.12, 57.375)
    mask_threshold: float = 0.0

    @property
    def grid(self) -> int:
        return self.img_size // self.patch_size


def preprocess_shape(h: int, w: int, L: int) -> Tuple[int, int]:
    sc = L * 1.0 / max(h, w)
    return int(h * sc + 0.5), int(w * sc + 0.5)


def resize_longest_side(img: np.ndarray, L: int) -> np.ndarray:
    from PIL import Image
    nh, nw = preprocess_shape(img.shape[0], img.shape[1], L)
    if (nh, nw) == img.shape[:2]:
        return np.ascontiguousarray(img)
    return np.asarray(Image.fromarray(img).resize((nw, nh), Image.BILINEAR))


MAX_TOKENS = 16


def _hyp(m: int) -> str:
    return "hyp" if m == 0 else f"m{m}hyp"


def check_prompts(point_coords=None, point_labels=None, boxes=None, mask_input=None,
                  mask_side: int = 256) -> Tuple[int, int]:
    def shape(t):
        return tuple(t.shape) if hasattr(t, "shape") else None

    def is_float(t):
        return (t.dtype.is_floating_point if isinstance(t.dtype, torch.dtype)
                else np.issubdtype(np.dtype(t.dtype), np.floating))

    def is_int_valued(t):
        if isinstance(t.dtype, torch.dtype):
            return not t.dtype.is_complex and t.dtype != torch.bool and (
                not t.dtype.is_floating_point or bool(torch.all(t == torch.round(t))))
        d = np.dtype(t.dtype)
        return np.issubdtype(d, np.integer) or (np.issubdtype(d, np.floating) and bool(np.all(t == np.round(t))))

    Ps = []
    n_sparse = 0
    if (point_coords is None) != (point_labels is None):
        raise ValueError("point_coords and point_labels must be given together")
    if point_coords is not None:
        sc, sl = shape(point_coords), shape(point_labels)
        if sc is None or len(sc) != 3 or sc[2] != 2 or not is_float(point_coords):
            raise ValueError(f"point_coords must be a float tensor [P, N, 2], got {sc}")
        if sl != sc[:2] or not is_int_valued(point_labels):
            raise ValueError(f"point_labels must be integer labels [P, N] = {list(sc[:2])}, got {sl}")
        Ps.append(sc[0])
        n_sparse += sc[1] + (1 if boxes is None else 0)
    if boxes is not None:
        sb = shape(boxes)
        if sb is None or len(sb) != 2 or sb[1] != 4 or not is_float(boxes):
            raise ValueError(f"boxes must be a float tensor [P, 4], got {sb}")
        Ps.append(sb[0])
        n_sparse += 2
    if mask_input is not None:
        sm = shape(mask_input)
        if sm is None or len(sm) != 4 or sm[1:] != (1, mask_side, mask_side) or not is_float(mask_input):
            raise ValueError(f"mask_input must be float low-res logits [P, 1, {mask_side}, {mask_side}], got {sm}")
        Ps.append(sm[0])
    P = Ps[0] if Ps else 1
    if any(p != P for p in Ps):
        raise ValueError(f"the prompts disagree on the batch size: {Ps}")
    if P < 1:
        raise ValueError("at least one prompt is needed")
    NT = 5 + n_sparse
    if NT > MAX_TOKENS:
        raise ValueError(f"{NT} decoder tokens per prompt (5 + {n_sparse} sparse) exceed the limit of {MAX_TOKENS}: "
                         f"at most 10 points without a box, or a box plus 9 points")
    return P, NT


class ResizeLongestSide:

    def __init__(self, target_length: int):
        self.target_length = target_length

    def apply_coords(self, coords: np.ndarray, original_size: Tuple[int, int]) -> np.ndarray:
        (oh, ow), (nh, nw) = original_size, preprocess_shape(original_size[0], original_size[1], self.target_length)
        c = np.array(coords, dtype=float)
        c[..., 0] = c[..., 0] * (nw / ow)
        c[..., 1] = c[..., 1] * (nh / oh)
        return c

    def apply_boxes(self, boxes: np.ndarray, original_size: Tuple[int, int]) -> np.ndarray:
        return self.apply_coords(np.asarray(boxes).reshape(-1, 2, 2), original_size).reshape(-1, 4)

    def apply_coords_torch(self, coords: torch.Tensor, original_size: Tuple[int, int]) -> torch.Tensor:
        (oh, ow), (nh, nw) = original_size, preprocess_shape(original_size[0], original_size[1], self.target_length)
        c = coords.detach().clone().to(torch.float)
        c[..., 0] = c[..., 0] * (nw / ow)
        c[..., 1] = c[..., 1] * (nh / oh)
        return c

    def apply_boxes_torch(self, boxes: torch.Tensor, original_size: Tuple[int, int]) -> torch.Tensor:
        return self.apply_coords_torch(boxes.reshape(-1, 2, 2), original_size).reshape(-1, 4)


def window_rows(B: int, g: int, ws: int) -> torch.Tensor:
    nwin = -(-g // ws)
    Mw = nwin * nwin * ws * ws
    r = torch.arange(B * Mw)
    b, rr = r // Mw, r % Mw
    win, pos = rr // (ws * ws), rr % (ws * ws)
    y = (win // nwin) * ws + pos // ws
    x = (win % nwin) * ws + pos % ws
    m = torch.where((y < g) & (x < g), b * g * g + y * g + x, torch.full_like(r, -1))
    return m.to(torch.int32)


def _to_dev_async(t: torch.Tensor, dev) -> torch.Tensor:
    return t.contiguous().pin_memory().to(dev, non_blocking=True)


class SamEngine:

    def __init__(self, state_dict: Dict[str, torch.Tensor], cfg: Optional[SamConfig] = None,
                 device: str | torch.device = "cuda", max_batch: int = 1, bias_correction: bool = True):
        cfg = cfg or SamConfig()
        self.cfg, self.dev = cfg, torch.device(device)
        assert self.dev.type == "cuda", "the InkLayer segmentor runs on MI355X only"
        D, g = cfg.embed_dim, cfg.grid
        assert D // cfg.num_heads == 80 and g == 64 and cfg.window_size == 14, \
            "HIP attention kernels are specialised for SAM's head_dim 80 / 64x64 grid / 14x14 windows"
        E = cfg.prompt_embed_dim
        assert E // cfg.dec_heads == 32 and (E // 2) // cfg.dec_heads == 16
        self.T = g * g
        assert E == 256 and (self.T * 4) % 32 == 0, \
            "the fused decoder kernels (csrc/proj_ln.hip, csrc/upscale_tail.hip) are built for SAM's widths"
        self.scale = 80 ** -0.5
        sd = state_dict
        dev = self.dev

        def h(name):
            return sd[name].detach().to(torch.float32).to(dev, F16).contiguous()

        def f(name):
            return ops.own_f32(sd[name], dev)

        def ws(name, shape=None):
            t = sd[name].detach().to(dev, torch.float32)
            return ops.split_weight(t if shape is None else shape(t))

        self.w: Dict[str, torch.Tensor] = {}
        w = self.w
        P = cfg.patch_size
        w["pe.ws"] = ws("image_encoder.patch_embed.proj.weight", lambda t: t.reshape(D, 3 * P * P))
        w["pe.b"] = f("image_encoder.patch_embed.proj.bias")
        w["pos"] = f("image_encoder.pos_embed").reshape(self.T, D).contiguous()
        for i in range(cfg.depth):
            p = f"image_encoder.blocks.{i}."
            for n in ("norm1.weight", "norm1.bias", "norm2.weight", "norm2.bias", "attn.qkv.bias",
                      "attn.proj.bias", "mlp.lin1.bias", "mlp.lin2.bias", "attn.rel_pos_h",
                      "attn.rel_pos_w"):
                w[f"b{i}.{n}"] = f(p + n)
            for n in ("attn.qkv.weight", "attn.proj.weight", "mlp.lin1.weight", "mlp.lin2.weight"):
                w[f"b{i}.{n}"] = h(p + n)
            if i not in cfg.global_attn_indexes:
                qb = w[f"b{i}.attn.qkv.bias"]
                w[f"b{i}.pad_k"] = qb[D:2 * D].to(F16).contiguous()
                w[f"b{i}.pad_v"] = qb[2 * D:].to(F16).contiguous()
        w["neck0.ws"] = ws("image_encoder.neck.0.weight", lambda t: t.reshape(E, D))
        w["neck1.w"], w["neck1.b"] = f("image_encoder.neck.1.weight"), f("image_encoder.neck.1.bias")
        w["neck2.ws"] = ws("image_encoder.neck.2.weight", lambda t: t.permute(0, 2, 3, 1).reshape(E, 9, E)) \
            .reshape(E, 27 * E).contiguous()
        w["neck3.w"], w["neck3.b"] = f("image_encoder.neck.3.weight"), f("image_encoder.neck.3.bias")

        w["gauss"] = f("prompt_encoder.pe_layer.positional_encoding_gaussian_matrix")
        w["no_mask"] = f("prompt_encoder.no_mask_embed.weight").reshape(-1).contiguous()
        w["pt_emb"] = torch.cat([f(f"prompt_encoder.point_embeddings.{i}.weight") for i in range(4)], 0).contiguous()
        if "prompt_encoder.not_a_point_embed.weight" in sd:
            w["not_a_point"] = f("prompt_encoder.not_a_point_embed.weight").reshape(-1).contiguous()
        md = "prompt_encoder.mask_downscaling."
        md_names = ("0.weight", "0.bias", "1.weight", "1.bias", "3.weight", "3.bias", "4.weight", "4.bias", "6.weight",
                    "6.bias")
        if all(md + n in sd for n in md_names):
            w["mask_ds"] = torch.cat([sd[md + n].detach().to(torch.float32).reshape(-1) for n in md_names]) \
                .to(dev).contiguous()
        ar = (torch.arange(g, dtype=torch.float32) + 0.5) / g
        grid_xy = torch.stack([ar[None, :].expand(g, g), ar[:, None].expand(g, g)], -1).reshape(-1, 2)
        self.dense_pe = ops.sam_pe_encode(grid_xy.contiguous().to(dev), w["gauss"])

        t = "mask_decoder.transformer."
        def attn(dst, src):
            for n in ("q_proj", "k_proj", "v_proj", "out_proj"):
                w[f"{dst}.{n}.ws"] = ws(f"{src}.{n}.weight")
                w[f"{dst}.{n}.b"] = f(f"{src}.{n}.bias")

        def cat(dst, names):
            for sfx in (".ws", ".b"):
                w[dst + sfx] = torch.cat([w[n + sfx] for n in names]).contiguous()

        pe_split = ops.add_split_f16(self.dense_pe)
        for i in range(cfg.dec_depth):
            p, d = f"{t}layers.{i}.", f"d{i}"
            attn(d + ".self", p + "self_attn")
            attn(d + ".t2i", p + "cross_attn_token_to_image")
            attn(d + ".i2t", p + "cross_attn_image_to_token")
            if i == 0:
                cat(d + ".self.qkv", [f"{d}.self.{n}" for n in ("q_proj", "k_proj", "v_proj")])
            else:
                cat(d + ".self.qk", [f"{d}.self.{n}" for n in ("q_proj", "k_proj")])
            for n in ("norm1", "norm2", "norm3", "norm4"):
                w[f"{d}.{n}.w"], w[f"{d}.{n}.b"] = f(p + n + ".weight"), f(p + n + ".bias")
            w[d + ".lin1.ws"], w[d + ".lin1.b"] = ws(p + "mlp.lin1.weight"), f(p + "mlp.lin1.bias")
            w[d + ".lin2.ws"], w[d + ".lin2.b"] = ws(p + "mlp.lin2.weight"), f(p + "mlp.lin2.bias")
            cat(d + ".kvq", [d + ".t2i.k_proj", d + ".t2i.v_proj", d + ".i2t.q_proj"])
            w[d + ".t2i.k_pe"] = ops.gemm(pe_split, w[d + ".t2i.k_proj.ws"]).contiguous()
            w[d + ".i2t.q_pe"] = ops.gemm(pe_split, w[d + ".i2t.q_proj.ws"]).contiguous()
            w[d + ".i2t.out_proj.blob"] = ops.proj256_ln_pack(w[d + ".i2t.out_proj.ws"].contiguous())
        attn("dfin", t + "final_attn_token_to_image")
        w["dfin.norm.w"], w["dfin.norm.b"] = f(t + "norm_final_attn.weight"), f(t + "norm_final_attn.bias")
        w["dfin.k_pe"] = ops.gemm(pe_split, w["dfin.k_proj.ws"]).contiguous()
        w["out_tok"] = torch.cat([f("mask_decoder.iou_token.weight"),
                                  f("mask_decoder.mask_tokens.weight")], 0).contiguous()
        u = "mask_decoder.output_upscaling."
        w["up0.ws"] = ws(u + "0.weight", lambda t: t.permute(2, 3, 1, 0).reshape(4 * (E // 4), E))
        w["up0.b"] = f(u + "0.bias").repeat(4).contiguous()
        w["up1.w"], w["up1.b"] = f(u + "1.weight"), f(u + "1.bias")
        up3 = ws(u + "3.weight", lambda t: t.permute(2, 3, 1, 0).reshape(4 * (E // 8), E // 4))
        assert tuple(up3.shape) == (128, 192)
        w["up3.blob"] = ops.sam_upscale_pack(up3.contiguous())
        w["up3.b"] = f(u + "3.bias").repeat(4).contiguous()
        cat("dfin.kvu", ["dfin.k_proj", "dfin.v_proj", "up0"])
        for j in range(3):
            w[f"iou{j}.ws"] = ws(f"mask_decoder.iou_prediction_head.layers.{j}.weight")
            w[f"iou{j}.b"] = f(f"mask_decoder.iou_prediction_head.layers.{j}.bias")
            for m in range(cfg.num_mask_tokens):
                hk = f"mask_decoder.output_hypernetworks_mlps.{m}.layers.{j}."
                if m == 0 or hk + "bias" in sd:
                    w[f"{_hyp(m)}{j}.b"] = f(hk + "bias")
                if m == 0 or hk + "weight" in sd:
                    w[f"{_hyp(m)}{j}.ws"] = ws(hk + "weight")

        self._alloc(max_batch)
        if bias_correction:
            self._calibrate_bias_correction(sd)

    @torch.no_grad()
    def _calibrate_bias_correction(self, sd) -> None:
        cfg, w, D = self.cfg, self.w, self.cfg.embed_dim
        page = torch.full((cfg.img_size, cfg.img_size, 3), 255, dtype=torch.uint8, device=self.dev)
        means: Dict[str, torch.Tensor] = {}
        self._calib = means
        try:
            self.encode([page])
        finally:
            self._calib = None
        for i in range(cfg.depth):
            p = f"image_encoder.blocks.{i}."
            for lin in ("attn.qkv", "mlp.lin1", "attn.proj", "mlp.lin2"):
                W32 = sd[p + lin + ".weight"].detach().to(self.dev, torch.float32)
                w16, bkey = w[f"b{i}.{lin}.weight"], f"b{i}.{lin}.bias"
                w[bkey] = (w[bkey].double() + (W32 - w16.float()).double() @ means[f"b{i}.{lin}"].double()).float().contiguous()

    def _alloc(self, B: int) -> None:
        cfg, dev, T, D = self.cfg, self.dev, self.T, self.cfg.embed_dim
        g, ws = cfg.grid, cfg.window_size
        self.max_batch = B
        nwin = -(-g // ws)
        self.nwin = nwin
        Mw = nwin * nwin * ws * ws
        self.Mw = Mw
        self._enc_graphs = LRU(self.graph_cache_size)
        self._enc_seen: Dict[int, int] = {}
        self.win_map = window_rows(B, g, ws).to(dev)
        P = cfg.patch_size
        e = lambda *s, dt=F16: torch.empty(s, device=dev, dtype=dt)
        self.buf_patches = e(B * T, 3 * P * P * 3)
        self.x = e(B * T, D, dt=F32)
        self.pos_rep = self.w["pos"].repeat(B, 1).contiguous()
        self.y = e(B * T, D)
        self.qkv = e(B * T, 3 * D)
        self.att = e(B * T, D)
        self.hid = e(B * T, int(D * cfg.mlp_ratio))
        H = cfg.num_heads
        self.rel_aug = e(B * nwin * nwin * H * ws * ws, 32)
        self.rel_h = e(B * H * T, 64)
        self.rel_w = e(B * H * T, 64)

    def encode(self, images_u8: Sequence[torch.Tensor], chan_reverse: bool = False,
               upto: Optional[int] = None) -> torch.Tensor:
        cfg, w, T, D = self.cfg, self.w, self.T, self.cfg.embed_dim
        B = len(images_u8)
        assert 1 <= B <= self.max_batch
        H, Mw = cfg.num_heads, self.Mw
        x = self.x[:B * T]
        for b, img in enumerate(images_u8):
            ops.sam_patchify(img, cfg.img_size, cfg.patch_size, cfg.pixel_mean, cfg.pixel_std,
                             chan_reverse, self.buf_patches[b * T:(b + 1) * T], split=True)
        ops.gemm(self.buf_patches[:B * T], w["pe.ws"], w["pe.b"], residual=self.pos_rep[:B * T], out=x)
        if upto is None and self.graph_blocks and ops.tracing_off():
            return self._blocks_graphed(B)
        return self._blocks(B, upto)

    graph_blocks = False
    graph_cache_size = 2

    def _blocks_graphed(self, B: int) -> torch.Tensor:
        g = self._enc_graphs.get(B)
        if g is None:
            self._enc_seen[B] = self._enc_seen.get(B, 0) + 1
            if self._enc_seen[B] < 2:
                return self._blocks(B, None)
            x0 = self.x[:B * self.T].clone()
            cur = torch.cuda.current_stream(self.dev)
            side = torch.cuda.Stream(device=self.dev)
            side.wait_stream(cur)
            with torch.cuda.stream(side):
                self._blocks(B, None)
                self.x[:B * self.T].copy_(x0)
            cur.wait_stream(side)
            graph = torch.cuda.CUDAGraph()
            with torch.cuda.graph(graph):
                out = self._blocks(B, None)
            self.x[:B * self.T].copy_(x0)
            g = (graph, out)
            self._enc_graphs.put(B, g)
        g[0].replay()
        return g[1].clone()

    def _blocks(self, B: int, upto: Optional[int]) -> torch.Tensor:
        cfg, w, T, D = self.cfg, self.w, self.T, self.cfg.embed_dim
        H, Mw = cfg.num_heads, self.Mw
        x = self.x[:B * T]
        nblk = cfg.depth if upto is None else upto
        calib = getattr(self, "_calib", None)
        for i in range(nblk):
            k = f"b{i}."
            y = ops.layernorm_rows(x, w[k + "norm1.weight"], w[k + "norm1.bias"], 1e-6, out=self.y[:B * T])
            if calib is not None:
                calib[k + "attn.qkv"] = y.float().mean(0)
            qkv = ops.gemm(y, w[k + "attn.qkv.weight"], w[k + "attn.qkv.bias"], out=self.qkv[:B * T])
            q, kk, v = qkv[:, :D], qkv[:, D:2 * D], qkv[:, 2 * D:]
            if i in cfg.global_attn_indexes:
                rh, rw = ops.relpos_bias(q, w[k + "attn.rel_pos_h"], w[k + "attn.rel_pos_w"], S=cfg.grid,
                                         n_batch=B, n_heads=H, head_dim=80, scale=self.scale,
                                         out=(self.rel_h, self.rel_w), f16_tables=True)
                o = ops.flash_attn(q, kk, v, n_batch=B, n_heads=H, head_dim=80, scale=self.scale,
                                   rel_h=rh, rel_w=rw, grid_w=cfg.grid, out=self.att[:B * T])
            else:
                wm = self.win_map[:B * Mw]
                nb = B * self.nwin * self.nwin
                aug = ops.relpos_bias(q, w[k + "attn.rel_pos_h"], w[k + "attn.rel_pos_w"],
                                      S=cfg.window_size, n_batch=nb, n_heads=H, head_dim=80,
                                      scale=self.scale, out=self.rel_aug, tok_rows=wm)
                o = ops.flash_attn(q, kk, v, n_batch=nb, n_heads=H, head_dim=80, scale=self.scale,
                                   n_q=cfg.window_size ** 2, n_k=cfg.window_size ** 2,
                                   rel_aug=aug, grid_w=cfg.window_size, tok_rows=wm,
                                   pad_k=w[k + "pad_k"], pad_v=w[k + "pad_v"], out=self.att[:B * T])
            if calib is not None:
                calib[k + "attn.proj"] = o.float().mean(0)
            ops.gemm(o, w[k + "attn.proj.weight"], w[k + "attn.proj.bias"], residual=x, out=x)
            y = ops.layernorm_rows(x, w[k + "norm2.weight"], w[k + "norm2.bias"], 1e-6, out=self.y[:B * T])
            hd = ops.gemm(y, w[k + "mlp.lin1.weight"], w[k + "mlp.lin1.bias"], act="gelu", out=self.hid[:B * T])
            if calib is not None:
                calib[k + "mlp.lin1"], calib[k + "mlp.lin2"] = y.float().mean(0), hd.float().mean(0)
            ops.gemm(hd, w[k + "mlp.lin2.weight"], w[k + "mlp.lin2.bias"], residual=x, out=x)
        if upto is not None:
            return x.view(B, T, D)
        n0 = ops.gemm(ops.add_split_f16(x), w["neck0.ws"])
        n1 = ops.layernorm_rows(n0, w["neck1.w"], w["neck1.b"], 1e-6, split=True)
        n2 = ops.gemm(ops.im2col3x3(n1, B, cfg.grid, cfg.grid), w["neck2.ws"])
        emb = ops.layernorm_rows(n2, w["neck3.w"], w["neck3.b"], 1e-6, out_dtype=F32)
        return emb.view(B, T, cfg.prompt_embed_dim)

    def decode(self, emb: torch.Tensor, boxes_input_frame: np.ndarray | torch.Tensor,
               input_hw: Tuple[int, int], orig_hw: Tuple[int, int], want_logits: bool = False):
        boxes = torch.as_tensor(np.asarray(boxes_input_frame), dtype=torch.float32).reshape(-1, 4)
        low, iou = self.decode_low_res(emb.reshape(1, self.T, -1), boxes, [0] * boxes.shape[0])
        res = ops.sam_postprocess(low, self.cfg.img_size, input_hw, orig_hw, self.cfg.mask_threshold, want_logits)
        if want_logits:
            return res[0], low, iou, res[1]
        return res

    def decode_low_res(self, emb: torch.Tensor, boxes: torch.Tensor, img_of_box: Sequence[int]):
        low, iou = self.decode_prompts(emb, img_of_box, boxes=boxes)
        return low.view(low.shape[0], *low.shape[-2:]), iou

    def decode_prompts(self, emb: torch.Tensor, img_of_prompt: Sequence[int], points: Optional[torch.Tensor] = None,
                       labels: Optional[torch.Tensor] = None, boxes: Optional[torch.Tensor] = None,
                       mask_input: Optional[torch.Tensor] = None, multimask_output: bool = False,
                       masks: Optional[Tuple[int, int]] = None):
        cfg, w, dev, L = self.cfg, self.w, self.dev, self.cfg.img_size
        P, _ = check_prompts(points, labels, boxes, mask_input, mask_side=4 * cfg.grid)
        if len(img_of_prompt) != P or not all(0 <= int(i) < emb.shape[0] for i in img_of_prompt):
            raise ValueError(f"img_of_prompt must name an image of emb for each of the {P} prompts")
        lo, M = masks if masks is not None else ((1, 3) if multimask_output else (0, 1))
        if M not in (1, 3, 4) or not 0 <= lo <= cfg.num_mask_tokens - M:
            raise ValueError(f"masks=(first, count) must select 1, 3 or 4 of the {cfg.num_mask_tokens} mask tokens")
        need = [("not_a_point", points is not None, "prompt_encoder.not_a_point_embed"),
                ("mask_ds", mask_input is not None, "prompt_encoder.mask_downscaling")]
        need += [(f"{_hyp(m)}0.ws", m > 0, f"mask_decoder.output_hypernetworks_mlps.{m}") for m in range(lo, lo + M)]
        missing = [name for key, used, name in need if used and key not in w]
        if missing:
            raise ValueError(f"these prompts need weights the engine's state dict did not have: {missing}")

        def dev32(t, dt=F32):
            t = torch.as_tensor(t)
            return t.to(dev, dt).contiguous() if t.is_cuda else _to_dev_async(t.to(dt), dev)

        pts = lab = bx = None
        if points is not None:
            pts, lab = dev32(points), dev32(labels, torch.int32)
        if boxes is not None:
            bx = dev32(torch.as_tensor(boxes).reshape(-1, 4))
        tokens = ops.sam_prompt_tokens(w["gauss"], w["pt_emb"], w.get("not_a_point", w["no_mask"]), w["out_tok"],
                                       float(L), P, points=pts, labels=lab, boxes=bx,
                                       pad=points is not None and boxes is None)
        mi = dev32(mask_input) if mask_input is not None else None
        return self._decode_tokens_split(emb, tokens, img_of_prompt, mask_input=mi, mask_lo=lo, n_masks=M)

    def _decode_tokens_split(self, emb: torch.Tensor, tokens: torch.Tensor, img_of_box: Sequence[int],
                             mask_input: Optional[torch.Tensor] = None, mask_lo: int = 0, n_masks: int = 1):
        cfg, w, T, dev = self.cfg, self.w, self.T, self.dev
        E, g = cfg.prompt_embed_dim, cfg.grid
        B = emb.shape[0]
        n, NT = tokens.shape[0], tokens.shape[1]
        assert n > 0 and len(img_of_box) == n and NT <= MAX_TOKENS
        Hh = cfg.dec_heads
        SP = ops.add_split_f16

        def lin(x_split, name, bias=True, **kw):
            return ops.gemm(x_split, w[name + ".ws"], w[name + ".b"] if bias else None, **kw)

        qpe = tokens.view(n * NT, E)
        iob = torch.as_tensor(list(img_of_box), dtype=torch.int64)
        img_rows = _to_dev_async((iob * T).to(torch.int32), dev)
        if mask_input is None:
            keys = ops.add_f32(emb.reshape(B * T, E).contiguous(), w["no_mask"])
            shared = True
            ks = None
        else:
            keys, ks = ops.sam_mask_embed(mask_input, emb.reshape(B * T, E).contiguous(), img_rows, w["mask_ds"], 1e-6,
                                          split=True)
            shared = False
        queries = qpe
        sc32, sc16 = 1.0 / math.sqrt(32), 1.0 / math.sqrt(16)

        Eh = E // 2

        def t2i_attend(name, queries, k, v, k_pe, residual):
            q = lin(SP(queries, qpe), name + ".q_proj")
            a = ops.attn_fewq(q, k, v, n_batch=n, n_heads=Hh, head_dim=16, scale=sc16, n_q=NT, n_k=T,
                              kv_batch_rows=img_rows if shared else None, k_add=k_pe)
            return lin(SP(a), name + ".out_proj", residual=residual)

        for i in range(cfg.dec_depth):
            d = f"d{i}"
            if i == 0:
                qkv = ops.gemm(SP(queries), w[d + ".self.qkv.ws"], w[d + ".self.qkv.b"])
                a = ops.attn_fewkeys(qkv[:, :E], qkv[:, E:2 * E], qkv[:, 2 * E:], B=n, n_heads=Hh, head_dim=32,
                                     scale=sc32)
                queries = lin(SP(a), d + ".self.out_proj")
            else:
                qk = ops.gemm(SP(queries, qpe), w[d + ".self.qk.ws"], w[d + ".self.qk.b"])
                v = lin(SP(queries), d + ".self.v_proj")
                a = ops.attn_fewkeys(qk[:, :E], qk[:, E:], v, B=n, n_heads=Hh, head_dim=32, scale=sc32)
                queries = lin(SP(a), d + ".self.out_proj", residual=queries)
            queries = ops.layernorm_rows(queries, w[d + ".norm1.w"], w[d + ".norm1.b"], 1e-5, out_dtype=F32)
            kvq = ops.gemm(SP(keys) if ks is None else ks, w[d + ".kvq.ws"], w[d + ".kvq.b"])
            queries = ops.layernorm_rows(t2i_attend(d + ".t2i", queries, kvq[:, :Eh], kvq[:, Eh:2 * Eh],
                                                    w[d + ".t2i.k_pe"], queries),
                                         w[d + ".norm2.w"], w[d + ".norm2.b"], 1e-5, out_dtype=F32)
            hmid = lin(SP(queries), d + ".lin1", act="relu")
            queries = ops.layernorm_rows(lin(SP(hmid), d + ".lin2", residual=queries),
                                         w[d + ".norm3.w"], w[d + ".norm3.b"], 1e-5, out_dtype=F32)
            ik = lin(SP(queries, qpe), d + ".i2t.k_proj")
            iv = lin(SP(queries), d + ".i2t.v_proj")
            a = ops.attn_fewkeys(kvq[:, 2 * Eh:], ik, iv, B=n, n_heads=Hh, head_dim=16, scale=sc16, n_q=T,
                                 q_batch_rows=img_rows if shared else None, q_add=w[d + ".i2t.q_pe"])
            last = i + 1 == cfg.dec_depth
            keys, ks = ops.proj256_ln(a, w[d + ".i2t.out_proj.blob"], w[d + ".i2t.out_proj.b"], keys, w[d + ".norm4.w"],
                                      w[d + ".norm4.b"], 1e-5, res_batch_rows=img_rows if shared else None,
                                      rows_per_batch=T if shared else 0, want_f32=not last, want_split=True)
            shared = False
        kvu = ops.gemm(ks, w["dfin.kvu.ws"], w["dfin.kvu.b"])
        kv = kvu[:, :2 * Eh]
        queries = ops.layernorm_rows(t2i_attend("dfin", queries, kv[:, :Eh], kv[:, Eh:], w["dfin.k_pe"], queries),
                                     w["dfin.norm.w"], w["dfin.norm.b"], 1e-5, out_dtype=F32)
        hs = queries.view(n, NT, E)

        def mlp3(prefix: str, x: torch.Tensor) -> torch.Tensor:
            a = lin(SP(x), prefix + "0", act="relu")
            a = lin(SP(a), prefix + "1", act="relu")
            return lin(SP(a), prefix + "2")

        M = n_masks
        if M == 1:
            hyper = mlp3(_hyp(mask_lo), hs[:, 1 + mask_lo].contiguous()).view(n, 1, 32)
        else:
            hyper = torch.stack([mlp3(_hyp(m), hs[:, 1 + m].contiguous()) for m in range(mask_lo, mask_lo + M)], 1)
        iou = mlp3("iou", hs[:, 0].contiguous())[:, mask_lo:mask_lo + M]
        u0 = kvu[:, 2 * Eh:]
        low = ops.sam_upscale_tail(u0, n, g, w["up1.w"], w["up1.b"], 1e-6, w["up3.blob"], w["up3.b"], hyper)
        return low, iou


class SamPredictor:

    def __init__(self, engine: SamEngine):
        self.engine = engine
        self.cfg = engine.cfg
        self.transform = ResizeLongestSide(engine.cfg.img_size)
        self.reset_image()

    def reset_image(self) -> None:
        self.is_image_set = False
        self.features = None
        self.original_size = None
        self.input_size = None

    def set_image(self, image: np.ndarray, image_format: str = "RGB") -> None:
        assert image_format in ("RGB", "BGR")
        if image_format != "RGB":
            image = image[..., ::-1]
        raw = torch.from_numpy(np.ascontiguousarray(image)).to(self.engine.dev)
        nh, nw = preprocess_shape(image.shape[0], image.shape[1], self.cfg.img_size)
        dev_img = ops.resize_bilinear_u8(raw, nh, nw)
        self.original_size = tuple(image.shape[:2])
        self.input_size = (nh, nw)
        self.features = self.engine.encode([dev_img])[0]
        self.is_image_set = True

    def apply_boxes(self, boxes: torch.Tensor) -> torch.Tensor:
        return self.transform.apply_boxes_torch(boxes.detach().cpu(), self.original_size)

    def apply_coords(self, coords: np.ndarray, original_size: Optional[Tuple[int, int]] = None) -> np.ndarray:
        return self.transform.apply_coords(coords, original_size or self.original_size)

    def apply_coords_torch(self, coords: torch.Tensor, original_size: Optional[Tuple[int, int]] = None) -> torch.Tensor:
        return self.transform.apply_coords_torch(coords, original_size or self.original_size)

    def predict(self, point_coords: Optional[np.ndarray] = None, point_labels: Optional[np.ndarray] = None,
                box: Optional[np.ndarray] = None, mask_input: Optional[np.ndarray] = None,
                multimask_output: bool = True, return_logits: bool = False):
        if not self.is_image_set:
            raise RuntimeError("An image must be set with .set_image(...) before mask prediction.")
        if point_coords is not None and point_labels is None:
            raise ValueError("point_labels must be supplied if point_coords is supplied.")
        coords = labels = boxes = mask = None
        if point_coords is not None:
            coords = torch.as_tensor(self.apply_coords(point_coords), dtype=torch.float)[None]
            labels = torch.as_tensor(np.asarray(point_labels), dtype=torch.int)[None]
        if box is not None:
            boxes = torch.as_tensor(self.transform.apply_boxes(box, self.original_size), dtype=torch.float)[:1]
        if mask_input is not None:
            mask = torch.as_tensor(mask_input, dtype=torch.float)[None]
        masks, iou, low = self.predict_torch(coords, labels, boxes, mask, multimask_output, return_logits=return_logits)
        return masks[0].cpu().numpy(), iou[0].cpu().numpy(), low[0].cpu().numpy()

    def predict_torch(self, point_coords=None, point_labels=None, boxes: torch.Tensor = None,
                      mask_input=None, multimask_output: bool = False, return_logits: bool = False):
        if not self.is_image_set:
            raise RuntimeError("An image must be set with .set_image(...) before mask prediction.")
        eng = self.engine
        P, _ = check_prompts(point_coords, point_labels, boxes, mask_input, mask_side=4 * self.cfg.grid)
        low, iou = eng.decode_prompts(self.features.reshape(1, eng.T, -1), [0] * P, point_coords, point_labels, boxes,
                                      mask_input, multimask_output)
        C, S = low.shape[1], low.shape[-1]
        res = ops.sam_postprocess(low.view(P * C, S, S), self.cfg.img_size, self.input_size, self.original_size,
                                  self.cfg.mask_threshold, return_logits)
        out = res[1] if return_logits else res.bool()
        return out.view(P, C, *self.original_size), iou, low


_ENGINES: Dict[str, SamEngine] = {}


def build_sam(checkpoint: Optional[str] = None, state_dict=None, device="cuda",
              max_batch: int = 1) -> SamEngine:
    if state_dict is None:
        if checkpoint in _ENGINES:
            return _ENGINES[checkpoint]
        state_dict = torch.load(checkpoint, map_location="cpu", weights_only=True)
    eng = SamEngine(state_dict, SamConfig(), device, max_batch)
    if checkpoint is not None:
        _ENGINES[checkpoint] = eng
    return eng


def run_SAM(image_pil, boxes_filt: torch.Tensor, sam_checkpoint: Optional[str] = None,
            engine: Optional[SamEngine] = None) -> List[np.ndarray]:
    if len(boxes_filt) == 0:
        return []
    eng = engine if engine is not None else build_sam(sam_checkpoint)
    pred = SamPredictor(eng)
    image = np.array(image_pil)[..., ::-1]
    pred.set_image(np.ascontiguousarray(image))
    tb = pred.apply_boxes(boxes_filt)
    masks, _, _ = pred.predict_torch(None, None, boxes=tb, multimask_output=False)
    m = masks[:, 0].cpu().numpy()
    return [m[i] for i in range(m.shape[0])]


def __getattr__(name):
    if name == "SamAutomaticMaskGenerator":
        from .amg import SamAutomaticMaskGenerator
        return SamAutomaticMaskGenerator
    raise AttributeError(f"module {__name__!r} has no attribute {name!r}")
```

Baseline: 121.0.

## Fuse SAM decoder token-path ops into three per-box megakernels

```diff
diff --git a/include/inklayer_hip.h b/include/inklayer_hip.h
--- a/include/inklayer_hip.h
+++ b/include/inklayer_hip.h
@@ -163,6 +163,14 @@
                          const void* blob_f16, const float* b3, const float* hyper, int32_t n_masks, float* low,
                          void* stream);
 
+int ink_sam_tokens_blob_floats(int32_t stage, int64_t* out_floats);
+int ink_sam_tokens_a(const float* queries, const float* qpe, const float* blob, int32_t layer0, int32_t n, int32_t n_tokens,
+                     float eps, float* queries_out, float* q_t2i, void* stream);
+int ink_sam_tokens_b(const float* queries, const float* qpe, const float* attn, const float* blob, int32_t n,
+                     int32_t n_tokens, float eps, float* queries_out, float* ik, float* iv, float* q_fin, void* stream);
+int ink_sam_tokens_c(const float* queries, const float* attn, const float* blob, int32_t n, int32_t n_tokens, float eps,
+                     int32_t mask_lo, int32_t n_masks, float* hs, float* iou, float* hyper, void* stream);
+
 int ink_proj256_ln_pack(const void* ws_f16, void* blob_f16, void* stream);
 int ink_proj256_ln(const float* a_f32, const void* blob_f16, const float* bias, const float* res_f32,
                    const int32_t* res_batch_rows, int32_t rows_per_batch, const float* ln_g, const float* ln_b, float eps,
diff --git a/inklayer_amd/_lib.py b/inklayer_amd/_lib.py
--- a/inklayer_amd/_lib.py
+++ b/inklayer_amd/_lib.py
@@ -92,6 +92,12 @@
     "ink_sam_upscale_pack": [c_void_p, c_void_p, c_void_p],
     "ink_sam_upscale_tail": [c_void_p, c_i64, c_int, c_int, c_void_p, c_void_p, c_float, c_void_p, c_void_p, c_void_p,
                              c_int, c_void_p, c_void_p],
+    "ink_sam_tokens_blob_floats": [c_int, C.POINTER(c_i64)],
+    "ink_sam_tokens_a": [c_void_p, c_void_p, c_void_p, c_int, c_int, c_int, c_float, c_void_p, c_void_p, c_void_p],
+    "ink_sam_tokens_b": [c_void_p, c_void_p, c_void_p, c_void_p, c_int, c_int, c_float, c_void_p, c_void_p, c_void_p,
+                         c_void_p, c_void_p],
+    "ink_sam_tokens_c": [c_void_p, c_void_p, c_void_p, c_int, c_int, c_float, c_int, c_int, c_void_p, c_void_p, c_void_p,
+                         c_void_p],
     "ink_ffn256_pack_bytes": [c_int, c_int, C.POINTER(c_i64)],
     "ink_ffn256_pack": [c_void_p, c_void_p, c_void_p, c_int, c_void_p, c_void_p, c_void_p],
     "ink_ffn256_fused": [c_void_p, c_i64, c_void_p, c_void_p, c_void_p, c_void_p, c_void_p, c_float, c_int, c_int,
diff --git a/inklayer_amd/build.py b/inklayer_amd/build.py
--- a/inklayer_amd/build.py
+++ b/inklayer_amd/build.py
@@ -23,7 +23,7 @@
     return max(h.stat().st_mtime for h in hs)
 
 
-NO_SPILL = {"ffn_fused.hip", "proj_ln.hip", "amg.hip"}
+NO_SPILL = {"ffn_fused.hip", "proj_ln.hip", "amg.hip", "sam_tokens.hip"}
 
 
 def _check_no_spill(src: Path, remarks: str) -> None:
diff --git a/inklayer_amd/csrc/sam_tokens.hip b/inklayer_amd/csrc/sam_tokens.hip
--- /dev/null
+++ b/inklayer_amd/csrc/sam_tokens.hip
@@ -0,0 +1,540 @@
+#include "common.h"
+
+namespace {
+
+constexpr int E = 256;
+constexpr int EH = 128;
+constexpr int HID = 2048;
+constexpr int CH = 1024;
+constexpr int NTH = 256;
+template <int TS>
+constexpr int kb_of() { return TS == 16 ? 8 : 16; }
+constexpr int RS = E + 4;
+constexpr int MAXR = 5;
+
+__device__ __forceinline__ f32x2 fma2(f32x2 a, f32x2 b, f32x2 c) { return __builtin_elementwise_fma(a, b, c); }
+
+template <bool WIDE>
+__device__ __forceinline__ f32x4 fetch_w(const float* __restrict__ W, int ldw, int k, int c) {
+  const float* r = W + (int64_t)k * ldw + c;
+  if (WIDE) return (f32x4){r[0], r[256], r[512], r[768]};
+  return *(const f32x4*)r;
+}
+
+template <int TS>
+__device__ __forceinline__ void fma_batch(f32x2 (&acc)[4][TS / 2], const f32x4 (&w)[kb_of<TS>()], const float* x) {
+  constexpr int KB = kb_of<TS>();
+#pragma unroll
+  for (int j = 0; j < KB; ++j) {
+#pragma unroll
+    for (int q = 0; q < TS / 4; ++q) {
+      const f32x4 xv = *(const f32x4*)(x + j * TS + 4 * q);
+      const f32x2 x01 = {xv.x, xv.y}, x23 = {xv.z, xv.w};
+#pragma unroll
+      for (int jj = 0; jj < 4; ++jj) {
+        const f32x2 ww = {w[j][jj], w[j][jj]};
+        acc[jj][2 * q] = fma2(x01, ww, acc[jj][2 * q]);
+        acc[jj][2 * q + 1] = fma2(x23, ww, acc[jj][2 * q + 1]);
+      }
+    }
+  }
+}
+
+template <int TS, bool WIDE>
+__device__ __forceinline__ void gemm_acc(f32x2 (&acc)[4][TS / 2], const float* x, const float* __restrict__ W, int ldw, int c,
+                                         int ks) {
+  constexpr int KB = kb_of<TS>();
+  f32x4 wa[KB], wb[KB];
+#pragma unroll
+  for (int j = 0; j < KB; ++j) wa[j] = fetch_w<WIDE>(W, ldw, j, c);
+  for (int k0 = 0; k0 < ks; k0 += 2 * KB) {
+#pragma unroll
+    for (int j = 0; j < KB; ++j) wb[j] = fetch_w<WIDE>(W, ldw, k0 + KB + j, c);
+    fma_batch<TS>(acc, wa, x + k0 * TS);
+    if (k0 + 2 * KB < ks) {
+#pragma unroll
+      for (int j = 0; j < KB; ++j) wa[j] = fetch_w<WIDE>(W, ldw, k0 + 2 * KB + j, c);
+    }
+    fma_batch<TS>(acc, wb, x + (k0 + KB) * TS);
+  }
+}
+
+template <int TS>
+__device__ __forceinline__ void zero_acc(f32x2 (&acc)[4][TS / 2]) {
+#pragma unroll
+  for (int jj = 0; jj < 4; ++jj)
+#pragma unroll
+    for (int q = 0; q < TS / 2; ++q) acc[jj][q] = (f32x2){0.0f, 0.0f};
+}
+
+template <int TS>
+__device__ __forceinline__ void store_part(const f32x2 (&acc)[4][TS / 2], float* part, int wave, int c0, bool active) {
+  if (!active) return;
+#pragma unroll
+  for (int q = 0; q < TS / 2; ++q) {
+    *(f32x4*)(part + (wave * TS + 2 * q) * E + c0) = (f32x4){acc[0][q].x, acc[1][q].x, acc[2][q].x, acc[3][q].x};
+    *(f32x4*)(part + (wave * TS + 2 * q + 1) * E + c0) = (f32x4){acc[0][q].y, acc[1][q].y, acc[2][q].y, acc[3][q].y};
+  }
+}
+
+template <int TS>
+__device__ __forceinline__ void gemm_part(const float* xa, const float* xb, const float* __restrict__ W, int ldw, int K,
+                                          int ncols, float* part) {
+  const int wave = threadIdx.x >> 6, lane = threadIdx.x & 63, c0 = 4 * lane;
+  const bool active = c0 < ncols;
+  const int ks = K >> 2;
+  f32x2 acc[4][TS / 2];
+  zero_acc<TS>(acc);
+  gemm_acc<TS, false>(acc, (lane < 32 ? xa : xb) + wave * ks * TS, W + (int64_t)wave * ks * ldw, ldw, active ? c0 : 0, ks);
+  store_part<TS>(acc, part, wave, c0, active);
+}
+
+__device__ __forceinline__ float part_sum(const float* part, int TS, int t, int c, float bias) {
+  const float* p = part + t * E + c;
+  return ((p[0] + p[TS * E]) + p[2 * TS * E]) + p[3 * TS * E] + bias;
+}
+
+template <int TS>
+__device__ __forceinline__ void block_ln(float (&v)[TS], float g, float b, float eps, float* red) {
+  const int wave = threadIdx.x >> 6, lane = threadIdx.x & 63;
+#pragma unroll
+  for (int t = 0; t < TS; ++t) {
+    const float s = wave_sum(v[t]);
+    if (lane == 0) red[wave * TS + t] = s;
+  }
+  __syncthreads();
+  float d[TS];
+#pragma unroll
+  for (int t = 0; t < TS; ++t)
+    d[t] = v[t] - (((red[t] + red[TS + t]) + red[2 * TS + t]) + red[3 * TS + t]) * (1.0f / E);
+  __syncthreads();
+#pragma unroll
+  for (int t = 0; t < TS; ++t) {
+    const float s = wave_sum(d[t] * d[t]);
+    if (lane == 0) red[wave * TS + t] = s;
+  }
+  __syncthreads();
+#pragma unroll
+  for (int t = 0; t < TS; ++t) {
+    const float var = (((red[t] + red[TS + t]) + red[2 * TS + t]) + red[3 * TS + t]) * (1.0f / E);
+    v[t] = fmaf(d[t] * (1.0f / sqrtf(var + eps)), g, b);
+  }
+  __syncthreads();
+}
+
+template <int TS>
+__device__ __forceinline__ void load_rows(float (&r)[TS], const float* __restrict__ src, int64_t row0, int nt, int ld, int c) {
+#pragma unroll
+  for (int t = 0; t < TS; ++t) r[t] = t < nt ? src[(row0 + t) * ld + c] : 0.0f;
+}
+
+template <int TS>
+__device__ __forceinline__ void put_col(float* xT, int c, const float (&r)[TS]) {
+#pragma unroll
+  for (int q = 0; q < TS / 4; ++q)
+    *(f32x4*)(xT + c * TS + 4 * q) = (f32x4){r[4 * q], r[4 * q + 1], r[4 * q + 2], r[4 * q + 3]};
+}
+
+constexpr int A_BQKV = E * 3 * E, A_WO = A_BQKV + 3 * E, A_BO = A_WO + E * E, A_G = A_BO + E, A_B = A_G + E,
+              A_WQ = A_B + E, A_BQ = A_WQ + E * EH, A_FLOATS = A_BQ + EH;
+
+template <int TS>
+constexpr int stage_a_lds_floats() { return 4 * TS * E + 2 * E * TS + 3 * TS * RS + 8 * 16 * 16 + 4 * TS; }
+
+template <int TS>
+__global__ __launch_bounds__(NTH) void sam_tokens_a_kernel(const float* __restrict__ queries, const float* __restrict__ qpe,
+                                                           const float* __restrict__ blob, int layer0, int nt, float eps,
+                                                           float* __restrict__ q_out, float* __restrict__ q_t2i) {
+  extern __shared__ __attribute__((aligned(16))) float lds[];
+  float* part = lds;
+  float* xq = part + 4 * TS * E;
+  float* xp = xq + E * TS;
+  float* rows = xp + E * TS;
+  float* sc = rows + 3 * TS * RS;
+  float* red = sc + 8 * 16 * 16;
+  const int c = threadIdx.x;
+  const int64_t row0 = (int64_t)blockIdx.x * nt;
+  float qr[TS], pe[TS], v[TS];
+  load_rows<TS>(qr, queries, row0, nt, E, c);
+  load_rows<TS>(pe, qpe, row0, nt, E, c);
+  put_col<TS>(xq, c, qr);
+#pragma unroll
+  for (int t = 0; t < TS; ++t) v[t] = layer0 ? qr[t] : qr[t] + pe[t];
+  put_col<TS>(xp, c, v);
+  __syncthreads();
+  for (int s = 0; s < 3; ++s) {
+    const float* x = s < 2 ? xp : xq;
+    gemm_part<TS>(x, x, blob + s * E, 3 * E, E, E, part);
+    __syncthreads();
+    const float bias = blob[A_BQKV + s * E + c];
+#pragma unroll
+    for (int t = 0; t < TS; ++t) rows[(s * TS + t) * RS + c] = part_sum(part, TS, t, c, bias);
+    __syncthreads();
+  }
+  const float scale = 0.17677669529663687f;
+  for (int i = c; i < 8 * nt * nt; i += NTH) {
+    const int h = i / (nt * nt), r = i - h * nt * nt, tq = r / nt, tk = r - tq * nt;
+    const float* qv = rows + tq * RS + h * 32;
+    const float* kv = rows + (TS + tk) * RS + h * 32;
+    float d = 0.0f;
+#pragma unroll
+    for (int e = 0; e < 32; e += 4) {
+      const f32x4 a = *(const f32x4*)(qv + e), b = *(const f32x4*)(kv + e);
+      d = fmaf(a.x, b.x, d);
+      d = fmaf(a.y, b.y, d);
+      d = fmaf(a.z, b.z, d);
+      d = fmaf(a.w, b.w, d);
+    }
+    sc[i] = d * scale;
+  }
+  __syncthreads();
+  {
+    const int h = c >> 5;
+    const float* vv = rows + 2 * TS * RS + c;
+#pragma unroll
+    for (int t = 0; t < TS; ++t) {
+      float o = 0.0f;
+      if (t < nt) {
+        const float* s = sc + (h * nt + t) * nt;
+        float m = s[0];
+        for (int tk = 1; tk < nt; ++tk) m = fmaxf(m, s[tk]);
+        float sum = 0.0f;
+        for (int tk = 0; tk < nt; ++tk) {
+          const float p = expf(s[tk] - m);
+          sum += p;
+          o = fmaf(p, vv[tk * RS], o);
+        }
+        o = o / sum;
+      }
+      v[t] = o;
+    }
+  }
+  put_col<TS>(xp, c, v);
+  __syncthreads();
+  gemm_part<TS>(xp, xp, blob + A_WO, E, E, E, part);
+  __syncthreads();
+  {
+    const float bias = blob[A_BO + c];
+#pragma unroll
+    for (int t = 0; t < TS; ++t) {
+      const float a = part_sum(part, TS, t, c, bias);
+      v[t] = layer0 ? a : qr[t] + a;
+    }
+  }
+  block_ln<TS>(v, blob[A_G + c], blob[A_B + c], eps, red);
+#pragma unroll
+  for (int t = 0; t < TS; ++t) {
+    if (t < nt) q_out[(row0 + t) * E + c] = v[t];
+    v[t] += pe[t];
+  }
+  put_col<TS>(xp, c, v);
+  __syncthreads();
+  gemm_part<TS>(xp, xp, blob + A_WQ, EH, E, EH, part);
+  __syncthreads();
+  if (c < EH) {
+    const float bias = blob[A_BQ + c];
+#pragma unroll
+    for (int t = 0; t < TS; ++t)
+      if (t < nt) q_t2i[(row0 + t) * EH + c] = part_sum(part, TS, t, c, bias);
+  }
+}
+
+constexpr int B_BOUT = EH * E, B_G2 = B_BOUT + E, B_B2 = B_G2 + E, B_W1 = B_B2 + E, B_B1 = B_W1 + E * HID,
+              B_W2 = B_B1 + HID, B_BL2 = B_W2 + HID * E, B_G3 = B_BL2 + E, B_B3 = B_G3 + E, B_WKV = B_B3 + E,
+              B_BKV = B_WKV + E * E, B_WQF = B_BKV + E, B_BQF = B_WQF + E * EH, B_FLOATS = B_WQF, B_FLOATS_FIN = B_BQF + EH;
+
+template <int TS>
+constexpr int stage_b_lds_floats() { return CH * TS + 3 * E * TS + 4 * TS; }
+
+template <int TS>
+__device__ __forceinline__ void load_a(float* xa, const float* __restrict__ a, int64_t row0, int nt, int c) {
+  if (c < EH) {
+    float r[TS];
+    load_rows<TS>(r, a, row0, nt, EH, c);
+    put_col<TS>(xa, c, r);
+  }
+}
+
+template <int TS>
+__global__ __launch_bounds__(NTH) void sam_tokens_b_kernel(const float* __restrict__ queries, const float* __restrict__ qpe,
+                                                           const float* __restrict__ a, const float* __restrict__ blob, int nt,
+                                                           float eps, float* __restrict__ q_out, float* __restrict__ ik,
+                                                           float* __restrict__ iv, float* __restrict__ q_fin) {
+  extern __shared__ __attribute__((aligned(16))) float lds[];
+  float* hT = lds;
+  float* part = lds;
+  float* xq = hT + CH * TS;
+  float* xp = xq + E * TS;
+  float* xa = xp + E * TS;
+  float* red = xa + E * TS;
+  const int c = threadIdx.x, wave = c >> 6, lane = c & 63;
+  const int64_t row0 = (int64_t)blockIdx.x * nt;
+  float qr[TS];
+  load_rows<TS>(qr, queries, row0, nt, E, c);
+  load_a<TS>(xa, a, row0, nt, c);
+  __syncthreads();
+  gemm_part<TS>(xa, xa, blob, E, EH, E, part);
+  __syncthreads();
+  {
+    const float bias = blob[B_BOUT + c];
+#pragma unroll
+    for (int t = 0; t < TS; ++t) qr[t] += part_sum(part, TS, t, c, bias);
+  }
+  block_ln<TS>(qr, blob[B_G2 + c], blob[B_B2 + c], eps, red);
+  put_col<TS>(xq, c, qr);
+  __syncthreads();
+  f32x2 acc2[4][TS / 2];
+  zero_acc<TS>(acc2);
+  for (int ch = 0; ch < HID / CH; ++ch) {
+    f32x2 acc1[4][TS / 2];
+    zero_acc<TS>(acc1);
+    gemm_acc<TS, true>(acc1, xq, blob + B_W1, HID, ch * CH + c, E);
+#pragma unroll
+    for (int jj = 0; jj < 4; ++jj) {
+      const float b1 = blob[B_B1 + ch * CH + c + 256 * jj];
+      float h[TS];
+#pragma unroll
+      for (int q = 0; q < TS / 2; ++q) {
+        h[2 * q] = fmaxf(acc1[jj][q].x + b1, 0.0f);
+        h[2 * q + 1] = fmaxf(acc1[jj][q].y + b1, 0.0f);
+      }
+      put_col<TS>(hT, c + 256 * jj, h);
+    }
+    __syncthreads();
+    gemm_acc<TS, false>(acc2, hT + wave * (CH / 4) * TS, blob + B_W2 + (int64_t)(ch * CH + wave * (CH / 4)) * E, E, 4 * lane,
+                        CH / 4);
+    __syncthreads();
+  }
+  store_part<TS>(acc2, part, wave, 4 * lane, true);
+  __syncthreads();
+  {
+    const float bias = blob[B_BL2 + c];
+#pragma unroll
+    for (int t = 0; t < TS; ++t) qr[t] = xq[c * TS + t] + part_sum(part, TS, t, c, bias);
+  }
+  block_ln<TS>(qr, blob[B_G3 + c], blob[B_B3 + c], eps, red);
+  put_col<TS>(xq, c, qr);
+  float pe[TS];
+  load_rows<TS>(pe, qpe, row0, nt, E, c);
+#pragma unroll
+  for (int t = 0; t < TS; ++t) {
+    if (t < nt) q_out[(row0 + t) * E + c] = qr[t];
+    pe[t] += qr[t];
+  }
+  put_col<TS>(xp, c, pe);
+  __syncthreads();
+  gemm_part<TS>(xp, xq, blob + B_WKV, E, E, E, part);
+  __syncthreads();
+  {
+    const float bias = blob[B_BKV + c];
+    float* dst = c < EH ? ik + c : iv + (c - EH);
+#pragma unroll
+    for (int t = 0; t < TS; ++t)
+      if (t < nt) dst[(row0 + t) * EH] = part_sum(part, TS, t, c, bias);
+  }
+  if (q_fin) {
+    __syncthreads();
+    gemm_part<TS>(xp, xp, blob + B_WQF, EH, E, EH, part);
+    __syncthreads();
+    if (c < EH) {
+      const float bias = blob[B_BQF + c];
+#pragma unroll
+      for (int t = 0; t < TS; ++t)
+        if (t < nt) q_fin[(row0 + t) * EH + c] = part_sum(part, TS, t, c, bias);
+    }
+  }
+}
+
+constexpr int C_BOUT = EH * E, C_G = C_BOUT + E, C_B = C_G + E, C_L0 = C_B + E, C_B0 = C_L0 + MAXR * E * E,
+              C_L1 = C_B0 + MAXR * E, C_B1 = C_L1 + MAXR * E * E, C_L2 = C_B1 + MAXR * E, C_B2 = C_L2 + MAXR * E * 32,
+              C_FLOATS = C_B2 + MAXR * 32;
+
+template <int TS>
+constexpr int stage_c_lds_floats() {
+  return (4 * TS * E > 4 * MAXR * E ? 4 * TS * E : 4 * MAXR * E) + 2 * E * TS + 2 * MAXR * E + 4 * TS;
+}
+
+__device__ __forceinline__ void gemv256(const float* x, int sk, int xo0, int xo_step, const float* __restrict__ W, int R,
+                                        int mask_lo, float* part) {
+  const int wave = threadIdx.x >> 6, lane = threadIdx.x & 63, k0 = wave * 64;
+  f32x4 acc[MAXR];
+#pragma unroll
+  for (int r = 0; r < MAXR; ++r) acc[r] = (f32x4){0.0f, 0.0f, 0.0f, 0.0f};
+  for (int kb = k0; kb < k0 + 64; kb += 8) {
+    f32x4 w[MAXR][8];
+#pragma unroll
+    for (int r = 0; r < MAXR; ++r)
+      if (r < R) {
+        const int wi = r == 0 ? 0 : mask_lo + r;
+#pragma unroll
+        for (int j = 0; j < 8; ++j) w[r][j] = *(const f32x4*)(W + ((int64_t)wi * E + kb + j) * E + 4 * lane);
+      }
+#pragma unroll
+    for (int r = 0; r < MAXR; ++r)
+      if (r < R) {
+        const int xo = r == 0 ? xo0 : xo0 + (mask_lo + r) * xo_step;
+#pragma unroll
+        for (int j = 0; j < 8; ++j) {
+          const float xv = x[(kb + j) * sk + xo];
+          acc[r].x = fmaf(xv, w[r][j].x, acc[r].x);
+          acc[r].y = fmaf(xv, w[r][j].y, acc[r].y);
+          acc[r].z = fmaf(xv, w[r][j].z, acc[r].z);
+          acc[r].w = fmaf(xv, w[r][j].w, acc[r].w);
+        }
+      }
+  }
+#pragma unroll
+  for (int r = 0; r < MAXR; ++r)
+    if (r < R) *(f32x4*)(part + (wave * MAXR + r) * E + 4 * lane) = acc[r];
+}
+
+template <int TS>
+__global__ __launch_bounds__(NTH) void sam_tokens_c_kernel(const float* __restrict__ queries, const float* __restrict__ a,
+                                                           const float* __restrict__ blob, int nt, float eps, int mask_lo,
+                                                           int M, float* __restrict__ hs_out, float* __restrict__ iou,
+                                                           float* __restrict__ hyper) {
+  extern __shared__ __attribute__((aligned(16))) float lds[];
+  constexpr int PART = 4 * TS * E > 4 * MAXR * E ? 4 * TS * E : 4 * MAXR * E;
+  float* part = lds;
+  float* xq = part + PART;
+  float* xa = xq + E * TS;
+  float* h0 = xa + E * TS;
+  float* h1 = h0 + MAXR * E;
+  float* red = h1 + MAXR * E;
+  const int c = threadIdx.x;
+  const int64_t row0 = (int64_t)blockIdx.x * nt;
+  const int R = 1 + M;
+  float qr[TS];
+  load_rows<TS>(qr, queries, row0, nt, E, c);
+  load_a<TS>(xa, a, row0, nt, c);
+  __syncthreads();
+  gemm_part<TS>(xa, xa, blob, E, EH, E, part);
+  __syncthreads();
+  {
+    const float bias = blob[C_BOUT + c];
+#pragma unroll
+    for (int t = 0; t < TS; ++t) qr[t] += part_sum(part, TS, t, c, bias);
+  }
+  block_ln<TS>(qr, blob[C_G + c], blob[C_B + c], eps, red);
+  put_col<TS>(xq, c, qr);
+  if (hs_out) {
+#pragma unroll
+    for (int t = 0; t < TS; ++t)
+      if (t < nt) hs_out[(row0 + t) * E + c] = qr[t];
+  }
+  __syncthreads();
+  gemv256(xq, TS, 0, 1, blob + C_L0, R, mask_lo, part);
+  __syncthreads();
+  for (int r = 0; r < R; ++r) {
+    const int wi = r == 0 ? 0 : mask_lo + r;
+    const float* p = part + r * E + c;
+    h0[wi * E + c] = fmaxf(((p[0] + p[MAXR * E]) + p[2 * MAXR * E]) + p[3 * MAXR * E] + blob[C_B0 + wi * E + c], 0.0f);
+  }
+  __syncthreads();
+  gemv256(h0, 1, 0, E, blob + C_L1, R, mask_lo, part);
+  __syncthreads();
+  for (int r = 0; r < R; ++r) {
+    const int wi = r == 0 ? 0 : mask_lo + r;
+    const float* p = part + r * E + c;
+    h1[wi * E + c] = fmaxf(((p[0] + p[MAXR * E]) + p[2 * MAXR * E]) + p[3 * MAXR * E] + blob[C_B1 + wi * E + c], 0.0f);
+  }
+  __syncthreads();
+  {
+    const int col = c & 31, sl = c >> 5;
+    for (int r = 0; r < R; ++r) {
+      const int wi = r == 0 ? 0 : mask_lo + r;
+      const float* w = blob + C_L2 + ((int64_t)wi * E + sl * 32) * 32 + col;
+      const float* x = h1 + wi * E + sl * 32;
+      float d = 0.0f;
+#pragma unroll
+      for (int k = 0; k < 32; ++k) d = fmaf(x[k], w[k * 32], d);
+      part[(r * 8 + sl) * 32 + col] = d;
+    }
+  }
+  __syncthreads();
+  if (c < R * 32) {
+    const int r = c >> 5, col = c & 31, wi = r == 0 ? 0 : mask_lo + r;
+    const float* p = part + r * 8 * 32 + col;
+    float s = p[0];
+#pragma unroll
+    for (int i = 1; i < 8; ++i) s += p[i * 32];
+    s += blob[C_B2 + wi * 32 + col];
+    if (r == 0) {
+      if (col < 4) iou[(int64_t)blockIdx.x * 4 + col] = s;
+    } else {
+      hyper[((int64_t)blockIdx.x * M + r - 1) * 32 + col] = s;
+    }
+  }
+}
+
+template <typename K>
+void allow_lds(K kernel, int bytes) {
+  (void)hipFuncSetAttribute((const void*)kernel, hipFuncAttributeMaxDynamicSharedMemorySize, bytes);
+}
+
+template <int TS>
+int launch_a(const float* q, const float* qpe, const float* blob, int layer0, int n, int nt, float eps, float* q_out,
+             float* q_t2i, hipStream_t stream) {
+  constexpr int bytes = stage_a_lds_floats<TS>() * 4;
+  static bool attr = (allow_lds(sam_tokens_a_kernel<TS>, bytes), true);
+  (void)attr;
+  hipLaunchKernelGGL(sam_tokens_a_kernel<TS>, dim3(n), dim3(NTH), bytes, stream, q, qpe, blob, layer0, nt, eps, q_out, q_t2i);
+  return ink_launch_status();
+}
+
+template <int TS>
+int launch_b(const float* q, const float* qpe, const float* a, const float* blob, int n, int nt, float eps, float* q_out,
+             float* ik, float* iv, float* q_fin, hipStream_t stream) {
+  constexpr int bytes = stage_b_lds_floats<TS>() * 4;
+  static bool attr = (allow_lds(sam_tokens_b_kernel<TS>, bytes), true);
+  (void)attr;
+  hipLaunchKernelGGL(sam_tokens_b_kernel<TS>, dim3(n), dim3(NTH), bytes, stream, q, qpe, a, blob, nt, eps, q_out, ik, iv, q_fin);
+  return ink_launch_status();
+}
+
+template <int TS>
+int launch_c(const float* q, const float* a, const float* blob, int n, int nt, float eps, int mask_lo, int M, float* hs,
+             float* iou, float* hyper, hipStream_t stream) {
+  constexpr int bytes = stage_c_lds_floats<TS>() * 4;
+  static bool attr = (allow_lds(sam_tokens_c_kernel<TS>, bytes), true);
+  (void)attr;
+  hipLaunchKernelGGL(sam_tokens_c_kernel<TS>, dim3(n), dim3(NTH), bytes, stream, q, a, blob, nt, eps, mask_lo, M, hs, iou, hyper);
+  return ink_launch_status();
+}
+
+inline bool aligned16(const void* p) { return ((uintptr_t)p & 15) == 0; }
+
+}
+
+extern "C" int ink_sam_tokens_blob_floats(int32_t stage, int64_t* out_floats) {
+  INK_CHECK_ARG(out_floats && stage >= 0 && stage <= 3);
+  *out_floats = stage == 0 ? A_FLOATS : stage == 1 ? B_FLOATS : stage == 2 ? B_FLOATS_FIN : C_FLOATS;
+  return INK_OK;
+}
+
+extern "C" int ink_sam_tokens_a(const float* queries, const float* qpe, const float* blob, int32_t layer0, int32_t n,
+                                int32_t n_tokens, float eps, float* queries_out, float* q_t2i, void* stream) {
+  INK_CHECK_ARG(n_tokens >= 1 && n_tokens <= 16 && n > 0);
+  INK_CHECK_ARG(queries && qpe && blob && queries_out && q_t2i && aligned16(blob));
+  const auto launch = n_tokens <= 8 ? launch_a<8> : launch_a<16>;
+  return launch(queries, qpe, blob, layer0 != 0, n, n_tokens, eps, queries_out, q_t2i, (hipStream_t)stream);
+}
+
+extern "C" int ink_sam_tokens_b(const float* queries, const float* qpe, const float* attn, const float* blob, int32_t n,
+                                int32_t n_tokens, float eps, float* queries_out, float* ik, float* iv, float* q_fin,
+                                void* stream) {
+  INK_CHECK_ARG(n_tokens >= 1 && n_tokens <= 16 && n > 0);
+  INK_CHECK_ARG(queries && qpe && attn && blob && queries_out && ik && iv && aligned16(blob));
+  const auto launch = n_tokens <= 8 ? launch_b<8> : launch_b<16>;
+  return launch(queries, qpe, attn, blob, n, n_tokens, eps, queries_out, ik, iv, q_fin, (hipStream_t)stream);
+}
+
+extern "C" int ink_sam_tokens_c(const float* queries, const float* attn, const float* blob, int32_t n, int32_t n_tokens,
+                                float eps, int32_t mask_lo, int32_t n_masks, float* hs, float* iou, float* hyper,
+                                void* stream) {
+  INK_CHECK_ARG(n_tokens >= 1 && n_tokens <= 16 && n > 0);
+  INK_CHECK_ARG(mask_lo >= 0 && n_masks >= 1 && mask_lo + n_masks <= 4 && 1 + mask_lo + n_masks <= n_tokens);
+  INK_CHECK_ARG(queries && attn && blob && iou && hyper && aligned16(blob));
+  const auto launch = n_tokens <= 8 ? launch_c<8> : launch_c<16>;
+  return launch(queries, attn, blob, n, n_tokens, eps, mask_lo, n_masks, hs, iou, hyper, (hipStream_t)stream);
+}
diff --git a/inklayer_amd/ops.py b/inklayer_amd/ops.py
--- a/inklayer_amd/ops.py
+++ b/inklayer_amd/ops.py
@@ -965,3 +965,102 @@
     check(_lib.lib().ink_im2col3x3_ex_f16(x.data_ptr(), B, H, W, Cn, stride, int(relu), out.data_ptr(), _stream()),
           "ink_im2col3x3_ex_f16")
     return out
+
+
+_SAM_T = "mask_decoder.transformer."
+
+
+def sam_tokens_blob_floats(stage: int) -> int:
+    n = C.c_int64()
+    check(_lib.lib().ink_sam_tokens_blob_floats(stage, C.byref(n)), "ink_sam_tokens_blob_floats")
+    return n.value
+
+
+def _sam_tokens_blob(parts: Sequence[torch.Tensor], stage: int) -> torch.Tensor:
+    blob = torch.cat([p.reshape(-1) for p in parts]).contiguous()
+    assert blob.dtype == F32 and blob.numel() == sam_tokens_blob_floats(stage), (blob.numel(), stage)
+    return blob
+
+
+def sam_tokens_pack(sd, dev, depth: int = 2, num_mask_tokens: int = 4):
+    def wt(name):
+        return sd[name + ".weight"].detach().to(dev, F32).t().contiguous()
+
+    def v(name):
+        return sd[name].detach().to(dev, F32).reshape(-1)
+
+    A, B = [], []
+    for i in range(depth):
+        p = f"{_SAM_T}layers.{i}."
+        sa, t2i, i2t = p + "self_attn.", p + "cross_attn_token_to_image.", p + "cross_attn_image_to_token."
+        A.append(_sam_tokens_blob([
+            torch.cat([wt(sa + n) for n in ("q_proj", "k_proj", "v_proj")], 1),
+            torch.cat([v(sa + n + ".bias") for n in ("q_proj", "k_proj", "v_proj")]),
+            wt(sa + "out_proj"), v(sa + "out_proj.bias"), v(p + "norm1.weight"), v(p + "norm1.bias"),
+            wt(t2i + "q_proj"), v(t2i + "q_proj.bias")], 0))
+        parts = [wt(t2i + "out_proj"), v(t2i + "out_proj.bias"), v(p + "norm2.weight"), v(p + "norm2.bias"),
+                 wt(p + "mlp.lin1"), v(p + "mlp.lin1.bias"), wt(p + "mlp.lin2"), v(p + "mlp.lin2.bias"),
+                 v(p + "norm3.weight"), v(p + "norm3.bias"),
+                 torch.cat([wt(i2t + "k_proj"), wt(i2t + "v_proj")], 1),
+                 torch.cat([v(i2t + "k_proj.bias"), v(i2t + "v_proj.bias")])]
+        last = i + 1 == depth
+        if last:
+            parts += [wt(_SAM_T + "final_attn_token_to_image.q_proj"), v(_SAM_T + "final_attn_token_to_image.q_proj.bias")]
+        B.append(_sam_tokens_blob(parts, 2 if last else 1))
+    fin = _SAM_T + "final_attn_token_to_image."
+    mlps = ["mask_decoder.iou_prediction_head.layers."] + \
+           [f"mask_decoder.output_hypernetworks_mlps.{m}.layers." for m in range(num_mask_tokens)]
+    parts = [wt(fin + "out_proj"), v(fin + "out_proj.bias"), v(_SAM_T + "norm_final_attn.weight"),
+             v(_SAM_T + "norm_final_attn.bias")]
+    for j, n_out in ((0, 256), (1, 256), (2, 32)):
+        ws, bs = [], []
+        for mp in mlps:
+            w_ = torch.zeros((256, n_out), device=dev, dtype=F32)
+            b_ = torch.zeros(n_out, device=dev, dtype=F32)
+            if f"{mp}{j}.weight" in sd and f"{mp}{j}.bias" in sd:
+                src = wt(f"{mp}{j}")
+                w_[:, :src.shape[1]] = src
+                b_[:src.shape[1]] = v(f"{mp}{j}.bias")
+            ws.append(w_)
+            bs.append(b_)
+        parts += [torch.stack(ws), torch.stack(bs)]
+    return A, B, _sam_tokens_blob(parts, 3)
+
+
+def _tok_rows(x: torch.Tensor, width: int) -> Tuple[int, int]:
+    assert x.dtype == F32 and x.is_contiguous() and x.dim() == 3 and x.shape[2] == width, (x.dtype, tuple(x.shape))
+    return x.shape[0], x.shape[1]
+
+
+def sam_tokens_a(queries: torch.Tensor, qpe: torch.Tensor, blob: torch.Tensor, layer0: bool, eps: float = 1e-5):
+    n, NT = _tok_rows(queries, 256)
+    assert _tok_rows(qpe, 256) == (n, NT) and blob.dtype == F32
+    q = torch.empty_like(queries)
+    qt = torch.empty((n, NT, 128), device=queries.device, dtype=F32)
+    check(_lib.lib().ink_sam_tokens_a(_p(queries), _p(qpe), _p(blob), int(layer0), n, NT, eps, _p(q), _p(qt), _stream()),
+          "ink_sam_tokens_a")
+    return q, qt
+
+
+def sam_tokens_b(queries: torch.Tensor, qpe: torch.Tensor, attn: torch.Tensor, blob: torch.Tensor, want_q_fin: bool,
+                 eps: float = 1e-5):
+    n, NT = _tok_rows(queries, 256)
+    assert _tok_rows(qpe, 256) == (n, NT) and _tok_rows(attn, 128) == (n, NT) and blob.dtype == F32
+    q = torch.empty_like(queries)
+    ik, iv = torch.empty_like(attn), torch.empty_like(attn)
+    qf = torch.empty_like(attn) if want_q_fin else None
+    check(_lib.lib().ink_sam_tokens_b(_p(queries), _p(qpe), _p(attn), _p(blob), n, NT, eps, _p(q), _p(ik), _p(iv), _p(qf),
+                                      _stream()), "ink_sam_tokens_b")
+    return q, ik, iv, qf
+
+
+def sam_tokens_c(queries: torch.Tensor, attn: torch.Tensor, blob: torch.Tensor, mask_lo: int, n_masks: int,
+                 eps: float = 1e-5, want_hs: bool = False):
+    n, NT = _tok_rows(queries, 256)
+    assert _tok_rows(attn, 128) == (n, NT) and blob.dtype == F32
+    iou = torch.empty((n, 4), device=queries.device, dtype=F32)
+    hyper = torch.empty((n, max(n_masks, 0), 32), device=queries.device, dtype=F32)
+    hs = torch.empty_like(queries) if want_hs else None
+    check(_lib.lib().ink_sam_tokens_c(_p(queries), _p(attn), _p(blob), n, NT, eps, mask_lo, n_masks, _p(hs), _p(iou),
+                                      _p(hyper), _stream()), "ink_sam_tokens_c")
+    return iou, hyper, hs
diff --git a/inklayer_amd/sam.py b/inklayer_amd/sam.py
--- a/inklayer_amd/sam.py
+++ b/inklayer_amd/sam.py
@@ -51,10 +51,6 @@
 
 
 MAX_TOKENS = 16
-
-
-def _hyp(m: int) -> str:
-    return "hyp" if m == 0 else f"m{m}hyp"
 
 
 def check_prompts(point_coords=None, point_labels=None, boxes=None, mask_input=None,
@@ -219,10 +215,9 @@
         self.dense_pe = ops.sam_pe_encode(grid_xy.contiguous().to(dev), w["gauss"])
 
         t = "mask_decoder.transformer."
-        def attn(dst, src):
-            for n in ("q_proj", "k_proj", "v_proj", "out_proj"):
-                w[f"{dst}.{n}.ws"] = ws(f"{src}.{n}.weight")
-                w[f"{dst}.{n}.b"] = f(f"{src}.{n}.bias")
+        def proj(dst, src):
+            w[f"{dst}.ws"] = ws(f"{src}.weight")
+            w[f"{dst}.b"] = f(f"{src}.bias")
 
         def cat(dst, names):
             for sfx in (".ws", ".b"):
@@ -231,23 +226,17 @@
         pe_split = ops.add_split_f16(self.dense_pe)
         for i in range(cfg.dec_depth):
             p, d = f"{t}layers.{i}.", f"d{i}"
-            attn(d + ".self", p + "self_attn")
-            attn(d + ".t2i", p + "cross_attn_token_to_image")
-            attn(d + ".i2t", p + "cross_attn_image_to_token")
-            if i == 0:
-                cat(d + ".self.qkv", [f"{d}.self.{n}" for n in ("q_proj", "k_proj", "v_proj")])
-            else:
-                cat(d + ".self.qk", [f"{d}.self.{n}" for n in ("q_proj", "k_proj")])
-            for n in ("norm1", "norm2", "norm3", "norm4"):
-                w[f"{d}.{n}.w"], w[f"{d}.{n}.b"] = f(p + n + ".weight"), f(p + n + ".bias")
-            w[d + ".lin1.ws"], w[d + ".lin1.b"] = ws(p + "mlp.lin1.weight"), f(p + "mlp.lin1.bias")
-            w[d + ".lin2.ws"], w[d + ".lin2.b"] = ws(p + "mlp.lin2.weight"), f(p + "mlp.lin2.bias")
+            proj(d + ".t2i.k_proj", p + "cross_attn_token_to_image.k_proj")
+            proj(d + ".t2i.v_proj", p + "cross_attn_token_to_image.v_proj")
+            proj(d + ".i2t.q_proj", p + "cross_attn_image_to_token.q_proj")
+            w[d + ".norm4.w"], w[d + ".norm4.b"] = f(p + "norm4.weight"), f(p + "norm4.bias")
             cat(d + ".kvq", [d + ".t2i.k_proj", d + ".t2i.v_proj", d + ".i2t.q_proj"])
             w[d + ".t2i.k_pe"] = ops.gemm(pe_split, w[d + ".t2i.k_proj.ws"]).contiguous()
             w[d + ".i2t.q_pe"] = ops.gemm(pe_split, w[d + ".i2t.q_proj.ws"]).contiguous()
-            w[d + ".i2t.out_proj.blob"] = ops.proj256_ln_pack(w[d + ".i2t.out_proj.ws"].contiguous())
-        attn("dfin", t + "final_attn_token_to_image")
-        w["dfin.norm.w"], w["dfin.norm.b"] = f(t + "norm_final_attn.weight"), f(t + "norm_final_attn.bias")
+            w[d + ".i2t.out_proj.blob"] = ops.proj256_ln_pack(ws(p + "cross_attn_image_to_token.out_proj.weight").contiguous())
+            w[d + ".i2t.out_proj.b"] = f(p + "cross_attn_image_to_token.out_proj.bias")
+        proj("dfin.k_proj", t + "final_attn_token_to_image.k_proj")
+        proj("dfin.v_proj", t + "final_attn_token_to_image.v_proj")
         w["dfin.k_pe"] = ops.gemm(pe_split, w["dfin.k_proj.ws"]).contiguous()
         w["out_tok"] = torch.cat([f("mask_decoder.iou_token.weight"),
                                   f("mask_decoder.mask_tokens.weight")], 0).contiguous()
@@ -260,15 +249,9 @@
         w["up3.blob"] = ops.sam_upscale_pack(up3.contiguous())
         w["up3.b"] = f(u + "3.bias").repeat(4).contiguous()
         cat("dfin.kvu", ["dfin.k_proj", "dfin.v_proj", "up0"])
-        for j in range(3):
-            w[f"iou{j}.ws"] = ws(f"mask_decoder.iou_prediction_head.layers.{j}.weight")
-            w[f"iou{j}.b"] = f(f"mask_decoder.iou_prediction_head.layers.{j}.bias")
-            for m in range(cfg.num_mask_tokens):
-                hk = f"mask_decoder.output_hypernetworks_mlps.{m}.layers.{j}."
-                if m == 0 or hk + "bias" in sd:
-                    w[f"{_hyp(m)}{j}.b"] = f(hk + "bias")
-                if m == 0 or hk + "weight" in sd:
-                    w[f"{_hyp(m)}{j}.ws"] = ws(hk + "weight")
+        self.tok_a, self.tok_b, self.tok_c = ops.sam_tokens_pack(sd, dev, cfg.dec_depth, cfg.num_mask_tokens)
+        self.hyper_tokens = [m for m in range(cfg.num_mask_tokens) if all(
+            f"mask_decoder.output_hypernetworks_mlps.{m}.layers.{j}.{k}" in sd for j in range(3) for k in ("weight", "bias"))]
 
         self._alloc(max_batch)
         if bias_correction:
@@ -428,8 +411,8 @@
             raise ValueError(f"masks=(first, count) must select 1, 3 or 4 of the {cfg.num_mask_tokens} mask tokens")
         need = [("not_a_point", points is not None, "prompt_encoder.not_a_point_embed"),
                 ("mask_ds", mask_input is not None, "prompt_encoder.mask_downscaling")]
-        need += [(f"{_hyp(m)}0.ws", m > 0, f"mask_decoder.output_hypernetworks_mlps.{m}") for m in range(lo, lo + M)]
         missing = [name for key, used, name in need if used and key not in w]
+        missing += [f"mask_decoder.output_hypernetworks_mlps.{m}" for m in range(lo, lo + M) if m not in self.hyper_tokens]
         if missing:
             raise ValueError(f"these prompts need weights the engine's state dict did not have: {missing}")
 
@@ -458,10 +441,7 @@
         Hh = cfg.dec_heads
         SP = ops.add_split_f16
 
-        def lin(x_split, name, bias=True, **kw):
-            return ops.gemm(x_split, w[name + ".ws"], w[name + ".b"] if bias else None, **kw)
-
-        qpe = tokens.view(n * NT, E)
+        qpe = tokens
         iob = torch.as_tensor(list(img_of_box), dtype=torch.int64)
         img_rows = _to_dev_async((iob * T).to(torch.int32), dev)
         if mask_input is None:
@@ -473,62 +453,34 @@
                                           split=True)
             shared = False
         queries = qpe
-        sc32, sc16 = 1.0 / math.sqrt(32), 1.0 / math.sqrt(16)
+        sc16 = 1.0 / math.sqrt(16)
 
         Eh = E // 2
 
-        def t2i_attend(name, queries, k, v, k_pe, residual):
-            q = lin(SP(queries, qpe), name + ".q_proj")
-            a = ops.attn_fewq(q, k, v, n_batch=n, n_heads=Hh, head_dim=16, scale=sc16, n_q=NT, n_k=T,
+        def t2i_attend(q, k, v, k_pe):
+            a = ops.attn_fewq(q.view(n * NT, Eh), k, v, n_batch=n, n_heads=Hh, head_dim=16, scale=sc16, n_q=NT, n_k=T,
                               kv_batch_rows=img_rows if shared else None, k_add=k_pe)
-            return lin(SP(a), name + ".out_proj", residual=residual)
+            return a.view(n, NT, Eh)
 
         for i in range(cfg.dec_depth):
             d = f"d{i}"
-            if i == 0:
-                qkv = ops.gemm(SP(queries), w[d + ".self.qkv.ws"], w[d + ".self.qkv.b"])
-                a = ops.attn_fewkeys(qkv[:, :E], qkv[:, E:2 * E], qkv[:, 2 * E:], B=n, n_heads=Hh, head_dim=32,
-                                     scale=sc32)
-                queries = lin(SP(a), d + ".self.out_proj")
-            else:
-                qk = ops.gemm(SP(queries, qpe), w[d + ".self.qk.ws"], w[d + ".self.qk.b"])
-                v = lin(SP(queries), d + ".self.v_proj")
-                a = ops.attn_fewkeys(qk[:, :E], qk[:, E:], v, B=n, n_heads=Hh, head_dim=32, scale=sc32)
-                queries = lin(SP(a), d + ".self.out_proj", residual=queries)
-            queries = ops.layernorm_rows(queries, w[d + ".norm1.w"], w[d + ".norm1.b"], 1e-5, out_dtype=F32)
+            last = i + 1 == cfg.dec_depth
+            queries, q_t2i = ops.sam_tokens_a(queries, qpe, self.tok_a[i], layer0=i == 0)
             kvq = ops.gemm(SP(keys) if ks is None else ks, w[d + ".kvq.ws"], w[d + ".kvq.b"])
-            queries = ops.layernorm_rows(t2i_attend(d + ".t2i", queries, kvq[:, :Eh], kvq[:, Eh:2 * Eh],
-                                                    w[d + ".t2i.k_pe"], queries),
-                                         w[d + ".norm2.w"], w[d + ".norm2.b"], 1e-5, out_dtype=F32)
-            hmid = lin(SP(queries), d + ".lin1", act="relu")
-            queries = ops.layernorm_rows(lin(SP(hmid), d + ".lin2", residual=queries),
-                                         w[d + ".norm3.w"], w[d + ".norm3.b"], 1e-5, out_dtype=F32)
-            ik = lin(SP(queries, qpe), d + ".i2t.k_proj")
-            iv = lin(SP(queries), d + ".i2t.v_proj")
+            a = t2i_attend(q_t2i, kvq[:, :Eh], kvq[:, Eh:2 * Eh], w[d + ".t2i.k_pe"])
+            queries, ik, iv, q_fin = ops.sam_tokens_b(queries, qpe, a, self.tok_b[i], want_q_fin=last)
+            ik, iv = ik.view(n * NT, Eh), iv.view(n * NT, Eh)
             a = ops.attn_fewkeys(kvq[:, 2 * Eh:], ik, iv, B=n, n_heads=Hh, head_dim=16, scale=sc16, n_q=T,
                                  q_batch_rows=img_rows if shared else None, q_add=w[d + ".i2t.q_pe"])
-            last = i + 1 == cfg.dec_depth
             keys, ks = ops.proj256_ln(a, w[d + ".i2t.out_proj.blob"], w[d + ".i2t.out_proj.b"], keys, w[d + ".norm4.w"],
                                       w[d + ".norm4.b"], 1e-5, res_batch_rows=img_rows if shared else None,
                                       rows_per_batch=T if shared else 0, want_f32=not last, want_split=True)
             shared = False
         kvu = ops.gemm(ks, w["dfin.kvu.ws"], w["dfin.kvu.b"])
         kv = kvu[:, :2 * Eh]
-        queries = ops.layernorm_rows(t2i_attend("dfin", queries, kv[:, :Eh], kv[:, Eh:], w["dfin.k_pe"], queries),
-                                     w["dfin.norm.w"], w["dfin.norm.b"], 1e-5, out_dtype=F32)
-        hs = queries.view(n, NT, E)
-
-        def mlp3(prefix: str, x: torch.Tensor) -> torch.Tensor:
-            a = lin(SP(x), prefix + "0", act="relu")
-            a = lin(SP(a), prefix + "1", act="relu")
-            return lin(SP(a), prefix + "2")
-
-        M = n_masks
-        if M == 1:
-            hyper = mlp3(_hyp(mask_lo), hs[:, 1 + mask_lo].contiguous()).view(n, 1, 32)
-        else:
-            hyper = torch.stack([mlp3(_hyp(m), hs[:, 1 + m].contiguous()) for m in range(mask_lo, mask_lo + M)], 1)
-        iou = mlp3("iou", hs[:, 0].contiguous())[:, mask_lo:mask_lo + M]
+        a = t2i_attend(q_fin, kv[:, :Eh], kv[:, Eh:], w["dfin.k_pe"])
+        iou, hyper, _ = ops.sam_tokens_c(queries, a, self.tok_c, mask_lo, n_masks)
+        iou = iou[:, mask_lo:mask_lo + n_masks]
         u0 = kvu[:, 2 * Eh:]
         low = ops.sam_upscale_tail(u0, n, g, w["up1.w"], w["up1.b"], 1e-6, w["up3.blob"], w["up3.b"], hyper)
         return low, iou
```

Result: slower. 119.2 (-1.5%).
